# Nyrox/raymond

Hardware: AMD Instinct MI355X
Metric: Msamples/s (whole node) + achieved HBM GB/s, 1920x1080 @ 500spp 5-bounce (higher is better)
Workload: dtype f64

## Files before the change

include/raymond_hip_probe.h:

```cpp
#ifndef RAYMOND_HIP_PROBE_H
#define RAYMOND_HIP_PROBE_H

#include "raymond_hip.h"

#ifdef __cplusplus
extern "C" {
#endif

rmd_status rmd_probe_philox4x32_10(rmd_context *ctx, size_t n, const uint32_t *ctr4, const uint32_t *key2, uint32_t *out4);
rmd_status rmd_probe_block_uniforms(rmd_context *ctx, uint64_t seed, size_t n, const uint32_t *pixel, const uint32_t *sample,
                                    const uint32_t *block, double *out5);
rmd_status rmd_probe_sphere_intersect(rmd_context *ctx, size_t n, const double *sphere4, const double *ray6, int32_t *hit, double *t);
rmd_status rmd_probe_sphere_normal(rmd_context *ctx, size_t n, const double *sphere4, const double *ray6, const double *t, double *n3);
rmd_status rmd_probe_plane_intersect(rmd_context *ctx, size_t n, const double *plane6, const double *ray6, int32_t *hit, double *t);
rmd_status rmd_probe_aabb_intersect(rmd_context *ctx, size_t n, const double *aabb6, const double *ray6, int32_t *hit, double *t);
rmd_status rmd_probe_triangle_intersect(rmd_context *ctx, size_t n, const double *pos9, const double *ray6, int32_t *hit, double *t);
rmd_status rmd_probe_triangle_normal(rmd_context *ctx, size_t n, const double *pos9, const double *nrm9, const double *ray6,
                                     const double *t, double *n3);
rmd_status rmd_probe_onb(rmd_context *ctx, size_t n, const double *n3, double *t3, double *b3);
rmd_status rmd_probe_cosine_hemisphere(rmd_context *ctx, size_t n, const double *r1, const double *r2, double *dir3, double *pdf);
rmd_status rmd_probe_importance_sample_ggx(rmd_context *ctx, size_t n, const double *reflect3, const double *rough, const double *r1,
                                           const double *r2, double *dir3);
rmd_status rmd_probe_ggx_distribution(rmd_context *ctx, size_t n, const double *n3, const double *h3, const double *rough, double *out);
rmd_status rmd_probe_geometry_smith(rmd_context *ctx, size_t n, const double *n3, const double *v3, const double *l3,
                                    const double *rough, double *out);
rmd_status rmd_probe_fresnel_schlick(rmd_context *ctx, size_t n, const double *cos_theta, const double *f0_3, double *out3);
rmd_status rmd_probe_elementary(rmd_context *ctx, size_t n, const double *x, double *sqrt_out, double *sin_out, double *cos_out,
                                double *root_out, double *inv_root_out);
rmd_status rmd_probe_primary_ray(rmd_context *ctx, size_t n, const rmd_camera *cam, const uint32_t *xy2, const double *u2, double *ray6);
rmd_status rmd_probe_scene_intersect(rmd_context *ctx, const rmd_scene *scene, size_t n, const double *ray6, int32_t *obj, double *t,
                                     uint32_t *sub);
rmd_status rmd_probe_grid_intersect(rmd_context *ctx, const rmd_scene *scene, uint32_t g, size_t n, const double *ray6, int32_t *hit,
                                    double *t, uint32_t *tri);
rmd_status rmd_probe_grid_intersect_deep(rmd_context *ctx, const rmd_scene *scene, uint32_t g, size_t n, const double *ray6, uint32_t cut_lanes,
                                         uint32_t cut_round, uint32_t rays_per_wave, int32_t *hit, double *t, uint32_t *tri);
rmd_status rmd_probe_trace_samples(rmd_context *ctx, const rmd_scene *scene, const rmd_camera *cam, const rmd_settings *settings,
                                   size_t n, const uint32_t *xy2, const uint32_t *sample, double *rgb_out, int32_t *path_obj,
                                   uint32_t *path_sub);

rmd_status rmd_probe_triangle_sphere(size_t n, const double *pos9, double *out5);
rmd_status rmd_probe_primary_candidates(const rmd_camera *cam, const rmd_settings *settings, const rmd_object *objects, uint32_t n_objects, uint32_t n_grids,
                                        int64_t axis_pairs_tunable, size_t n_tiles, const uint32_t *tiles4, uint64_t *launch3, uint64_t *out2);
rmd_status rmd_probe_launch_plan(uint32_t mode, uint32_t grid, size_t n, const uint32_t *in5, uint64_t *out8);
rmd_status rmd_probe_launch_sizes(uint32_t mode, uint32_t grid, uint64_t *out8);
rmd_status rmd_probe_work_plan(const rmd_context *ctx, size_t n, const uint32_t *in4, uint32_t *out3);
rmd_status rmd_probe_work_items(uint32_t n_tiles, uint32_t n_whole, uint32_t k_tail, uint32_t sample_count, uint32_t first, size_t n, uint32_t *out5,
                                uint32_t *n_items);
rmd_status rmd_probe_scene_layout(const rmd_scene *scene, uint32_t *n_objects, uint32_t *n_grids, uint32_t *mask_words_total);
rmd_status rmd_probe_scene_plan(const rmd_scene *scene, uint64_t *out8, size_t n, uint32_t *shift_bits2);
#define RMD_PROBE_SCRATCH_FORMS 7u
#define RMD_PROBE_SCRATCH_PARTS 15u
rmd_status rmd_probe_denoise_scratch(uint32_t form, uint32_t width, uint32_t height, uint32_t n_rects, uint32_t guided, uint32_t n_cands, uint64_t n_table,
                                     uint64_t *out3, uint64_t *total);
rmd_status rmd_probe_denoise_scratch_slope(uint32_t form, uint32_t width, uint32_t height, uint32_t n_rects, uint32_t guided, uint32_t sloped, uint32_t n_cands,
                                           uint64_t n_table, uint64_t *out3, uint64_t *total);
rmd_status rmd_probe_denoise_tile(uint32_t radius, uint32_t patch_radius, uint64_t *out4);
rmd_status rmd_probe_feature_slope(rmd_context *ctx, const double *fplanes7, uint32_t width, uint32_t height, double slope, double *mplanes7);
rmd_status rmd_probe_atrous_region_slope_planes(rmd_context *ctx, uint32_t width, uint32_t height, double *mplanes7);
rmd_status rmd_probe_pretest_pairs(rmd_context *ctx, size_t n, const double *sphere5, const double *pos9, const double *ray6, int32_t *pass,
                                   int32_t *hit, double *t);

#ifdef __cplusplus
}
#endif
#endif
```

raymond_amd/csrc/api.cpp:

```cpp
#define RMD_WITH_HIP 1
#include <algorithm>
#include <cmath>
#include <limits>
#include <cstddef>
#include <cstdio>
#include <cstdlib>
#include <cstring>
#include <new>

#include "internal.hpp"
#include "launch.hpp"
#include "luma_bins.hpp"
#include "resolve_tiles_host.hpp"

using rmd::bind;

namespace {
thread_local std::string tl_last_error;

rmd_status context_create(int32_t device, hipStream_t stream, bool own_stream, rmd_context **out) {
	if (!out) return rmd::fail(nullptr, RMD_ERR_INVALID_ARGUMENT, "rmd_context_create: null out pointer");
	*out = nullptr;
	int count = 0;
	hipError_t e = hipGetDeviceCount(&count);
// ... 87 lines not shown
		RMD_HIP(ctx, hipMemcpyAsync(ctx->wave_tiles.as<rmd::WaveTile>(), wt.data(), wt.size() * sizeof(rmd::WaveTile), hipMemcpyHostToDevice, ctx->stream));
		RMD_HIP(ctx, hipStreamSynchronize(ctx->stream));
	}
	ctx->n_wave_tiles = (uint32_t)wt.size();
	ctx->cached_rects.assign(tiles, tiles + n_tiles);
	ctx->cached_W = W, ctx->cached_H = H;
	return RMD_OK;
}

rmd_status check_render_args(rmd_context *ctx, const rmd_scene *scene, const rmd_camera *cam, const rmd_settings *st) {
	if (!scene || !cam || !st) return rmd::fail(ctx, RMD_ERR_INVALID_ARGUMENT, "render: null scene/camera/settings");
	if (scene->ctx != ctx) return rmd::fail(ctx, RMD_ERR_INVALID_ARGUMENT, "render: scene belongs to another context");
	if (cam->backbuffer_width == 0 || cam->backbuffer_height == 0 || cam->backbuffer_width > 65535u || cam->backbuffer_height > 65535u)
		return rmd::fail(ctx, RMD_ERR_INVALID_ARGUMENT, "render: backbuffer size must be 1..65535 per axis");
	if (st->bounce_limit > RMD_MAX_BOUNCE_LIMIT) return rmd::fail(ctx, RMD_ERR_UNSUPPORTED, "render: bounce_limit above RMD_MAX_BOUNCE_LIMIT");
	if ((uint64_t)st->sample_begin + st->sample_count > 0xFFFFFFFFull) return rmd::fail(ctx, RMD_ERR_INVALID_ARGUMENT, "render: sample range overflows u32");
	if (st->flags & ~(RMD_RENDER_DOF | RMD_RENDER_TRACE_BLACK_PATHS | RMD_RENDER_END_BLACK_PATHS)) return rmd::fail(ctx, RMD_ERR_INVALID_ARGUMENT, "render: unknown bits in rmd_settings.flags");
	if ((st->flags & RMD_RENDER_TRACE_BLACK_PATHS) && (st->flags & RMD_RENDER_END_BLACK_PATHS))
		return rmd::fail(ctx, RMD_ERR_INVALID_ARGUMENT, "render: RMD_RENDER_TRACE_BLACK_PATHS and RMD_RENDER_END_BLACK_PATHS exclude each other");
	if (rmd::render_lds_bytes(scene->n_objects, scene->mask_words_total, 1) + (scene->n_grids == 0u ? rmd::kSortPoolBytes : 0u) > rmd::kLdsBudgetBytes)
		return rmd::fail(ctx, RMD_ERR_UNSUPPORTED, "render: object table + grid masks exceed the 160 KiB LDS of a CU");
	return RMD_OK;
}

}

namespace rmd {

rmd_status fail(rmd_context *ctx, rmd_status status, const std::string &text) {
	if (ctx) ctx->last_error = text;
	tl_last_error = text;
	return status;
}

rmd_status fail_noexcept(rmd_context *ctx, rmd_status status, const char *what, const char *text) noexcept {
	try {
		return fail(ctx, status, std::string(what) + ": " + text);
	} catch (...) {
		try {
			if (ctx) ctx->last_error.clear();
			tl_last_error.clear();
		} catch (...) {
		}
		return status;
	}
}

rmd_status bind(rmd_context *ctx) {
	if (!ctx) return fail(nullptr, RMD_ERR_INVALID_ARGUMENT, "null context");
	RMD_HIP(ctx, hipSetDevice(ctx->device));
	return RMD_OK;
}

static_assert(RMD_MAX_BOUNCE_LIMIT_DEV == RMD_MAX_BOUNCE_LIMIT, "launch.hpp mirrors include/raymond_hip.h");

rmd_status check_fault(rmd_context *ctx) {
	if (!ctx || !ctx->h_fault) return RMD_OK;
	volatile uint32_t *f = ctx->h_fault;
	const uint32_t code = f[0];
	if (code == 0u) return RMD_OK;
	const uint32_t item = f[1], reports = f[2];
	f[0] = 0u, f[1] = 0u, f[2] = 0u;
	std::string what;
	if (code & kFaultTripLoop) what += " trip loop of render_wave;";
	if (code & kFaultSortedTripLoop) what += " trip loop of render_wave_sorted;";
	if (code & kFaultWorkLoop) what += " work loop of a persistent workgroup;";
	if (code & kFaultWalkRounds) what += " round loop of a grid walk;";
	if (code & kFaultQueuedTripLoop) what += " trip loop of render_wave_queued;";
	if (code & ~(kFaultTripLoop | kFaultSortedTripLoop | kFaultWorkLoop | kFaultWalkRounds | kFaultQueuedTripLoop)) what += " unknown code;";
	char num[96];
	std::snprintf(num, sizeof(num), " %u wave(s) reported, the last one at work item %u (code 0x%x)", reports, item, code);
	return fail(ctx, RMD_ERR_DEVICE_FAULT,
	            "device fault: a loop of the render kernel ran past its bound —" + what + num +
	                "; the launch was cut short and the framebuffer it wrote to is not valid");
}

bool primary_cull_allowed(const RenderParams &P) {
	CullCamera c;
	for (int a = 0; a < 3; a++) c.pos[a] = P.cam_pos[a];
	c.width = P.width, c.height = P.height, c.aspect = P.aspect, c.tan_half_fov = P.tan_half_fov;
	return P.use_dof == 0u && cull_camera_ok(c);
}

static bool camera_on_a_plane(const rmd_scene *scene, const rmd_camera *cam) {
	for (size_t i = 0; i + 6 <= scene->planes.size(); i += 6) {
		const double *o = &scene->planes[i], *n = o + 3;
		double num = 0.0, scale = 0.0;
		for (int a = 0; a < 3; a++) num += (o[a] - cam->position[a]) * -n[a], scale += (std::fabs(o[a]) + std::fabs(cam->position[a])) * std::fabs(n[a]);
		if (!(std::fabs(num) > 1e-9 * scale)) return true;
	}
	return false;
}

RenderParams make_params(const rmd_context *ctx, const rmd_scene *scene, const rmd_camera *cam, const rmd_settings *st) {
	const double PI = 3.14159265358979323846;
	RenderParams P;
	std::memset(&P, 0, sizeof(P));
	for (int a = 0; a < 3; a++) P.cam_pos[a] = cam->position[a];
	P.width = (double)cam->backbuffer_width;
	P.height = (double)cam->backbuffer_height;
	P.inv_width = rmd::exact_reciprocal(P.width), P.inv_height = rmd::exact_reciprocal(P.height);
	P.aspect = P.width / P.height;
	P.tan_half_fov = std::tan(cam->fov_vert / 2.0 * PI / 180.0);
	P.focal_length = cam->focal_length;
	P.aperture_radius = cam->aperture_radius;
	P.W = cam->backbuffer_width, P.H = cam->backbuffer_height;
	P.bounce_limit = st->bounce_limit;
	P.sample_begin = st->sample_begin, P.sample_count = st->sample_count;
	P.n_objects = scene ? scene->n_objects : 0;
	P.n_grids = scene ? scene->n_grids : 0;
	P.mask_words_total = scene ? scene->mask_words_total : 0;
	P.key0 = (uint32_t)st->seed, P.key1 = (uint32_t)(st->seed >> 32);
	P.use_dof = ((st->flags & RMD_RENDER_DOF) && cam->aperture_radius > 0.0) ? 1u : 0u;
	const bool on_plane = scene && camera_on_a_plane(scene, cam);
	P.end_black_paths = (st->flags & RMD_RENDER_TRACE_BLACK_PATHS) ? 0u : ((st->flags & RMD_RENDER_END_BLACK_PATHS) || !scene || (scene->n_grids == 0u && scene->regular && !on_plane)) ? 1u : 0u;
	P.shade_last_depth = (scene && (!scene->regular || on_plane)) ? 1u : 0u;
	P.axis_pairs = scene ? scene->axis_pairs : 0u;
	P.visit_mask = scene ? scene->visit_mask : ~0ull, P.grid_mask = scene ? scene->grid_mask : ~0ull;
	P.primary_cull = (scene && scene->primary_cull && rmd::primary_cull_allowed(P)) ? 1u : 0u;
	P.fault = ctx ? ctx->d_fault : nullptr;
	P.walk_batch = rmd::kWalkBatchDefault;
	if (ctx && ctx->tunable[RMD_TUNE_WALK_BATCH] > 0) P.walk_batch = (uint32_t)ctx->tunable[RMD_TUNE_WALK_BATCH];
	{
		uint32_t k = rmd::kWalkCutDefault;
		if (ctx && ctx->tunable[RMD_TUNE_WALK_CUT] > 0) k = (uint32_t)std::min<int64_t>(ctx->tunable[RMD_TUNE_WALK_CUT] - 1, 31);
		P.walk_cut = (scene && scene->n_grid_objects == 1u) ? (k | (2u * k) << 8) : 0u;
		P.walk_steps_bound = scene ? scene->walk_steps_bound : 0u;
	}
#if RMD_DIAG
	if (ctx) P.debug_flags = ctx->debug_flags;
#endif
	return P;
}

}

extern "C" {

uint32_t rmd_abi_version(void) { return RMD_ABI_VERSION; }

rmd_status rmd_context_create(int32_t device_ordinal, rmd_context **out) { return context_create(device_ordinal, nullptr, true, out); }

rmd_status rmd_context_create_on_stream(int32_t device_ordinal, void *hip_stream, rmd_context **out) {
	return context_create(device_ordinal, (hipStream_t)hip_stream, false, out);
}

rmd_context::~rmd_context() {
	(void)hipSetDevice(device);
	if (stream || !owns_stream) (void)hipStreamSynchronize(stream);
	if (h_fault) (void)hipHostFree(h_fault);
	if (copy_stream) (void)hipStreamSynchronize(copy_stream);
	for (auto &sl : transfer) {
		if (sl.packed_ready) (void)hipEventDestroy(sl.packed_ready);
		if (sl.copied) (void)hipEventDestroy(sl.copied);
	}
	if (copy_stream) (void)hipStreamDestroy(copy_stream);
	if (ev_start) (void)hipEventDestroy(ev_start);
	if (ev_stop) (void)hipEventDestroy(ev_stop);
	if (owns_stream && stream) (void)hipStreamDestroy(stream);
}

void rmd_context_destroy(rmd_context *ctx) { delete ctx; }

const char *rmd_last_error(const rmd_context *ctx) { return ctx ? ctx->last_error.c_str() : tl_last_error.c_str(); }

struct GridDerived {
	std::vector<unsigned char> recs;
	std::vector<rmd::CellEntry> entries;
	std::vector<uint32_t> ids;
	std::vector<double> aux;
	std::vector<double> spheres;
	double sphere_kb = 0.0;
};
static rmd_status derive_grid_tables(rmd_context *ctx, const rmd_grid_desc &g, GridDerived &out) {
	{
		if (!g.cells || !g.mapping_table || !g.tri_pos || !g.tri_nrm || g.n_tris == 0 ||
		    g.n_cells != (uint64_t)g.resolution[0] * g.resolution[1] * g.resolution[2]) {
			return rmd::fail(ctx, RMD_ERR_INVALID_ARGUMENT, "rmd_scene_create: inconsistent grid description");
		}
		for (uint64_t c = 0; c < g.n_cells; c++) {
			uint64_t off = g.cells[c];
			if (off >= g.n_mapping || off + (uint64_t)g.mapping_table[off] >= g.n_mapping) {
				return rmd::fail(ctx, RMD_ERR_INVALID_ARGUMENT, "rmd_scene_create: cells/mapping_table run out of range");
			}
			uint32_t cnt = g.mapping_table[off];
			for (uint32_t k = 1; k <= cnt; k++)
				if (g.mapping_table[off + k] >= g.n_tris) {
					return rmd::fail(ctx, RMD_ERR_INVALID_ARGUMENT, "rmd_scene_create: triangle index out of range in mapping_table");
				}
		}
		if ((uint64_t)g.resolution[0] * ((uint64_t)g.resolution[1] + (uint64_t)g.resolution[2] * g.resolution[2]) >= (1ull << 31) ||
		    g.n_cells > (1ull << 31)) {
			return rmd::fail(ctx, RMD_ERR_UNSUPPORTED, "rmd_scene_create: grid resolution too large for 31-bit cell indices");
		}
		const uint64_t n_refs = g.n_mapping - g.n_cells;
		if (n_refs > 0xFFFFFFFFull) {
			return rmd::fail(ctx, RMD_ERR_UNSUPPORTED, "rmd_scene_create: more than 2^32-1 cell->triangle references");
		}
		std::vector<unsigned char> &recs = out.recs;
		recs.assign((size_t)g.n_tris * rmd::kTriRecStride, 0);
		for (uint64_t ti = 0; ti < g.n_tris; ti++) {
			const double *p = g.tri_pos + (size_t)ti * 9;
// ... 79 lines not shown
		if (o.material.kind != RMD_MAT_EMISSION && o.material.roughness != 0.0 && std::fabs(o.material.roughness) < rmd::kMinRoughness)
			return rmd::fail(ctx, RMD_ERR_UNSUPPORTED, "rmd_scene_create: 0 < |roughness| < 1e-12 is not supported");
		d.roughness = o.material.roughness;
		d.metalness = o.material.kind == RMD_MAT_METAL ? 1.0 : 0.0;
		{
			auto tame = [](double v) { return std::fabs(v) <= 1e150; };
			bool ok = true;
			if (o.geometry_kind != RMD_GEOM_GRID)
				for (int a = 0; a < 3; a++) ok = ok && tame(o.origin[a]);
			if (o.geometry_kind == RMD_GEOM_PLANE)
				for (int a = 0; a < 3; a++) ok = ok && tame(o.normal[a]);
			if (o.geometry_kind == RMD_GEOM_SPHERE) ok = ok && tame(o.radius) && o.radius != 0.0 && o.radius * o.radius > 0.0;
			for (int a = 0; a < 3; a++) ok = ok && tame(o.material.color[a]);
			if (o.material.kind != RMD_MAT_EMISSION) ok = ok && tame(o.material.roughness) && o.material.roughness != 0.0;
			regular = regular && ok;
		}
		if (o.material.kind == RMD_MAT_DIFFUSE && o.material.color[0] == 0.0 && o.material.color[1] == 0.0 && o.material.color[2] == 0.0) d.flags |= rmd::kObjBlackDiffuse;
	}
	for (uint32_t j = 0; j < n_objects; j++) {
		if (hobj[j].geometry_kind != RMD_GEOM_PLANE) continue;
		for (uint32_t i = 0; i < j; i++) {
			if (hobj[i].geometry_kind != RMD_GEOM_PLANE || hobj[i].pair_info != 0u) continue;
			bool opposite = true;
			for (int a = 0; a < 3; a++) opposite = opposite && hobj[j].normal[a] == -hobj[i].normal[a];
			if (!opposite) continue;
			hobj[i].pair_info = rmd::kPairTestedAtPartner | j, hobj[j].pair_info = i + 1u;
			break;
		}
	}
	uint32_t axis_pairs = 0;
	for (uint32_t j = 0; j < n_objects && j < 1023u && regular && axis_pairs_tunable != 1; j++) {
		if (hobj[j].geometry_kind != RMD_GEOM_PLANE || hobj[j].pair_info == 0u || (hobj[j].pair_info & rmd::kPairTestedAtPartner)) continue;
		const uint32_t i = hobj[j].pair_info - 1u;
		int k = -1, nonzero = 0;
		for (int a = 0; a < 3; a++)
			if (hobj[i].normal[a] != 0.0) nonzero++, k = a;
		if (nonzero != 1 || (hobj[i].normal[k] != 1.0 && hobj[i].normal[k] != -1.0) || ((axis_pairs >> (10 * k)) & 1023u) != 0u) continue;
		axis_pairs |= (j + 1u) << (10 * k);
		hobj[j].flags |= rmd::kObjAxisPair | ((uint32_t)k << rmd::kObjAxisShift) | (hobj[i].normal[k] == 1.0 ? rmd::kObjAxisEarlierIsPlus : 0u);
		hobj[i].flags |= rmd::kObjAxisPair;
		hobj[j].partner_origin_k = hobj[i].origin[k];
		hobj[j].pair_info = rmd::kPairTestedAtPartner | rmd::kPairAxis | i;
		hobj[i].pair_info |= rmd::kPairAxis;
	}
	{
		rmd::AxisWalls *walls = out.walls;
		std::memset(walls, 0, 3 * sizeof(rmd::AxisWalls));
		for (int k = 0; k < 3; k++) {
			const uint32_t f = (axis_pairs >> (10 * k)) & 1023u;
			if (f == 0u) continue;
			const uint32_t j = f - 1u, i = hobj[j].pair_info & 0x3FFFFFFFu;
			const bool e_plus = (hobj[j].flags & rmd::kObjAxisEarlierIsPlus) != 0u;
			walls[k].o_plus = e_plus ? hobj[i].origin[k] : hobj[j].origin[k], walls[k].o_minus = e_plus ? hobj[j].origin[k] : hobj[i].origin[k];
			walls[k].idx_plus = e_plus ? i : j, walls[k].idx_minus = e_plus ? j : i;
		}
	}
	out.visit_mask = 0ull, out.grid_mask = 0ull;
	for (uint32_t i = 0; i < n_objects && i < 64u; i++) {
		if (!(hobj[i].geometry_kind == RMD_GEOM_PLANE && (hobj[i].pair_info & rmd::kPairTestedAtPartner))) out.visit_mask |= 1ull << i;
		if (hobj[i].geometry_kind == RMD_GEOM_GRID) out.grid_mask |= 1ull << i;
	}
	out.regular = regular, out.axis_pairs = axis_pairs;
	return RMD_OK;
}

static rmd_status scene_create_impl(rmd_context *ctx, const rmd_object *objects, uint32_t n_objects, const rmd_grid_desc *grids, uint32_t n_grids,
                                    rmd_scene **out) {
	if (rmd_status s = bind(ctx)) return s;
	if (!out || (n_objects && !objects) || (n_grids && !grids)) return rmd::fail(ctx, RMD_ERR_INVALID_ARGUMENT, "rmd_scene_create: null argument");
	rmd::SceneObjects derived;
	if (rmd_status s = rmd::derive_scene_objects(ctx, objects, n_objects, n_grids, ctx->tunable[RMD_TUNE_AXIS_PAIRS], derived)) return s;
	std::vector<rmd::DevObject> &hobj = derived.objs;
	const bool regular = derived.regular;
	const uint32_t axis_pairs = derived.axis_pairs;
	auto sc = std::make_unique<rmd_scene>();
	sc->ctx = ctx, sc->n_objects = n_objects, sc->n_grids = n_grids, sc->regular = regular;
	sc->axis_pairs = axis_pairs;
	rmd::DevObject walls_block;
	std::memset(&walls_block, 0, sizeof(walls_block));
	std::memcpy(&walls_block, derived.walls, sizeof(derived.walls));
	sc->visit_mask = derived.visit_mask, sc->grid_mask = derived.grid_mask;
	for (uint32_t i = 0; i < n_objects; i++)
		if (objects[i].geometry_kind == RMD_GEOM_PLANE) sc->planes.insert(sc->planes.end(), objects[i].origin, objects[i].origin + 3), sc->planes.insert(sc->planes.end(), objects[i].normal, objects[i].normal + 3);
	sc->primary_cull = regular && n_grids == 0u && ctx->tunable[RMD_TUNE_AXIS_PAIRS] == 0;
	for (uint32_t i = 0; i < n_objects; i++) sc->n_grid_objects += objects[i].geometry_kind == RMD_GEOM_GRID ? 1u : 0u;
	auto upload = [&](const void *src, size_t bytes, void **dst) -> hipError_t {
		*dst = nullptr;
		rmd::DeviceBuffer b;
		hipError_t e = b.alloc(bytes ? bytes : 16);
		if (e != hipSuccess) return e;
		*dst = b.as<void>();
		sc->owned.push_back(std::move(b));
		if (bytes) e = hipMemcpy(*dst, src, bytes, hipMemcpyHostToDevice);
		return e;
	};
	std::vector<rmd::DevGrid> hgrid(n_grids);
	for (uint32_t gi = 0; gi < n_grids; gi++) {
		const rmd_grid_desc &g = grids[gi];
		rmd::DevGrid &d = hgrid[gi];
		std::memset(&d, 0, sizeof(d));
		std::shared_ptr<const GridDerived> derived;
		{
			rmd_grid_build *gb = const_cast<rmd_grid_build *>(g.built);
			const bool from_build = gb && gb->cells.data() == g.cells && gb->cells.size() == g.n_cells && gb->mapping.data() == g.mapping_table &&
			                        gb->mapping.size() == g.n_mapping && gb->pos.data() == g.tri_pos && gb->nrm.data() == g.tri_nrm && gb->pos.size() == g.n_tris * 9;
			std::unique_lock<std::mutex> lock;
			if (from_build) {
				lock = std::unique_lock<std::mutex>(gb->derived_mutex);
				derived = std::static_pointer_cast<const GridDerived>(gb->derived);
			}
			if (!derived) {
				auto fresh = std::make_shared<GridDerived>();
				if (rmd_status st = derive_grid_tables(ctx, g, *fresh)) return st;
				derived = fresh;
				if (from_build) gb->derived = fresh;
			}
		}
		const std::vector<unsigned char> &recs = derived->recs;
		const std::vector<rmd::CellEntry> &entries = derived->entries;
		const std::vector<uint32_t> &ids = derived->ids;
		const std::vector<double> &aux = derived->aux;
		for (int a = 0; a < 3; a++) {
			d.bbox_min[a] = g.bbox_min[a], d.bbox_max[a] = g.bbox_max[a], d.cell_size[a] = g.cell_size[a];
			d.inv_cell_size[a] = rmd::exact_reciprocal(g.cell_size[a]);
			d.res[a] = g.resolution[a];
			if (a == 2) sc->walk_steps_bound = std::max<uint32_t>(sc->walk_steps_bound, (uint32_t)std::min<uint64_t>((uint64_t)g.resolution[0] + g.resolution[1] + g.resolution[2] + 3u, 0xFFFFFFFFull));
		}
		d.n_cells = g.n_cells, d.n_tris = g.n_tris;
		uint64_t last_nonempty = 0;
		bool any_nonempty = false;
		for (uint64_t c = 0; c < g.n_cells; c++)
			if (entries[c * rmd::kEntrySlots].count) last_nonempty = c, any_nonempty = true;
		uint64_t covered = any_nonempty ? last_nonempty + 1 : 0;
		size_t budget_bytes = rmd::kMaskBudgetBytes;
		if (ctx->tunable[RMD_TUNE_MASK_BUDGET] > 0) budget_bytes = (size_t)ctx->tunable[RMD_TUNE_MASK_BUDGET];
		if (budget_bytes < 64) budget_bytes = 64;
		if (budget_bytes > rmd::kMaskBudgetBytes) budget_bytes = rmd::kMaskBudgetBytes;
		const size_t budget_words = budget_bytes / 4 / n_grids;
		if (budget_words < 2)
			return rmd::fail(ctx, RMD_ERR_UNSUPPORTED, "rmd_scene_create: too many grids for the LDS occupancy-mask budget");
		if ((g.n_cells + 31) / 32 + 1 <= budget_words) covered = g.n_cells;
		uint32_t shift = 0;
		while (shift < 63 && ((covered >> shift) + 31) / 32 + 1 > budget_words) shift++;
		const uint64_t bits = covered ? ((covered - 1) >> shift) + 1 : 0;
		std::vector<uint32_t> mask((size_t)((bits + 31) / 32) + 1, 0u);
		for (uint64_t c = 0; c < covered; c++)
			if (entries[c * rmd::kEntrySlots].count) mask[(c >> shift) >> 5] |= 1u << ((c >> shift) & 31u);
		d.mask_bits = (uint32_t)bits, d.mask_shift = shift, d.mask_n_words = (uint32_t)mask.size();
		d.mask_lds_word = sc->mask_words_total;
		sc->mask_words_total += (uint32_t)((mask.size() + 3) & ~(size_t)3);
		void *p = nullptr;
		RMD_HIP(ctx, upload(entries.data(), entries.size() * sizeof(rmd::CellEntry), &p));
		d.cell_entries = (const rmd::CellEntry *)p;
		RMD_HIP(ctx, upload(ids.data(), ids.size() * sizeof(uint32_t), &p));
		d.tri_ids = (const uint32_t *)p;
		RMD_HIP(ctx, upload(recs.data(), recs.size(), &p));
		d.tri_recs = p;
		RMD_HIP(ctx, upload(mask.data(), mask.size() * sizeof(uint32_t), &p));
		d.mask_words = (const uint32_t *)p;
		RMD_HIP(ctx, upload(g.tri_pos, g.n_tris * 9 * sizeof(double), &p));
		d.tri_pos = (const double *)p;
		RMD_HIP(ctx, upload(g.tri_nrm, g.n_tris * 9 * sizeof(double), &p));
		d.tri_nrm = (const double *)p;
		RMD_HIP(ctx, upload(aux.data(), aux.size() * sizeof(double), &p));
		d.tri_aux = (const double *)p;
		RMD_HIP(ctx, upload(derived->spheres.data(), derived->spheres.size() * sizeof(double), &p));
		d.tri_sph = (const double *)p, d.sph_kb = derived->sphere_kb;
// ... 53 lines not shown
}
rmd_status rmd_framebuffer_upload(rmd_context *ctx, const double *host, double *dev, size_t n) {
	if (rmd_status s = bind(ctx)) return s;
	if (!dev || !host) return rmd::fail(ctx, RMD_ERR_INVALID_ARGUMENT, "rmd_framebuffer_upload: null pointer");
	RMD_HIP(ctx, hipMemcpyAsync(dev, host, n * sizeof(double), hipMemcpyHostToDevice, ctx->stream));
	RMD_HIP(ctx, hipStreamSynchronize(ctx->stream));
	return RMD_OK;
}

static uint32_t choose_split(const rmd_context *ctx, bool has_grid, uint32_t n_wave_tiles, uint32_t sample_count, bool *buffered = nullptr) {
	uint32_t k = 1;
	bool may_buffer_unsplit = n_wave_tiles != 0 && sample_count >= (has_grid ? 1u : rmd::kSortedMinSamples);
	if (ctx->tunable[RMD_TUNE_SAMPLE_SPLIT] > 0) {
		k = (uint32_t)ctx->tunable[RMD_TUNE_SAMPLE_SPLIT];
		if (k > sample_count / 4u) k = sample_count / 4u;
		may_buffer_unsplit = false;
	} else if (n_wave_tiles != 0) {
		const uint32_t waves_per_slot = has_grid ? 256u : 24u;
		k = (waves_per_slot * ctx->wave_slots + n_wave_tiles - 1u) / n_wave_tiles;
		if (has_grid && k < 2u) k = 2u;
		uint32_t min_samples = has_grid ? (sample_count <= rmd::kChainMaxSamples && ctx->tunable[RMD_TUNE_CHAIN_ITEMS] != 1 ? 2u : rmd::kSplitMinSamplesGrid) : 64u;
		if (ctx->tunable[RMD_TUNE_SPLIT_MIN_SAMPLES] > 0) min_samples = (uint32_t)std::min<int64_t>(ctx->tunable[RMD_TUNE_SPLIT_MIN_SAMPLES], 1 << 20);
		if (k > sample_count / min_samples) k = sample_count / min_samples;
		if (has_grid && k < 2u && sample_count >= 4u && ctx->tunable[RMD_TUNE_SPLIT_MIN_SAMPLES] <= 0) k = 2u;
	}
	if (k > 64u) k = 64u;
	while (k > 1u && (uint64_t)n_wave_tiles * k > 0x7FFFFFFFull) k--;
	if (k < 2u) k = 1u;
	if (buffered) *buffered = k > 1u || may_buffer_unsplit;
	return k;
}

extern "C++" {
namespace rmd {
WorkPlan plan_work_list(uint32_t wave_slots, uint32_t n_tiles, uint32_t sample_count, uint32_t k_uniform, uint32_t min_samples, uint32_t tail_x2, uint32_t tail_parts,
                        uint32_t n_tail_forced) {
	WorkPlan w{0u, n_tiles, k_uniform < 1u ? 1u : k_uniform};
	if (tail_x2 == 0u || sample_count > kWholeMaxSamples) return w;
	const uint64_t n_tail = n_tail_forced ? (uint64_t)n_tail_forced : ((uint64_t)tail_x2 * wave_slots + 1u) / 2u;
	if ((uint64_t)n_tiles <= n_tail) return w;
	uint32_t k = tail_parts > 64u ? 64u : tail_parts;
	if (min_samples < 1u) min_samples = 1u;
	if (k > sample_count / min_samples) k = sample_count / min_samples;
	if (k < w.k_tail) k = w.k_tail;
	if ((uint64_t)(n_tiles - n_tail) + n_tail * k > 0x7FFFFFFFull) return w;
	w.n_whole = n_tiles - (uint32_t)n_tail, w.n_tail = (uint32_t)n_tail, w.k_tail = k;
	return w;
}
static WorkPlan pass_work_plan(const rmd_context *ctx, bool has_grid, bool split_launch, bool buffered, bool persistent, uint32_t n_tiles, uint32_t sample_count,
                               bool *persistent_pass) {
	WorkPlan w{0u, n_tiles, split_launch ? choose_split(ctx, has_grid, n_tiles, sample_count) : 1u};
	*persistent_pass = persistent && ((uint64_t)n_tiles * w.k_tail >= ctx->wave_slots || ctx->tunable[RMD_TUNE_LAUNCH_FORM] == 2);
	if (!buffered || has_grid || !*persistent_pass || ctx->tunable[RMD_TUNE_SAMPLE_SPLIT] > 0) return w;
	uint32_t min_samples = kTailMinSamples, forced_tail = 0u;
	if (ctx->tunable[RMD_TUNE_SPLIT_MIN_SAMPLES] > 0) min_samples = (uint32_t)std::min<int64_t>(ctx->tunable[RMD_TUNE_SPLIT_MIN_SAMPLES], 1 << 20);
#if RMD_DIAG
	if (ctx->debug_flags & 1024u) forced_tail = 4u;
#endif
	return plan_work_list(ctx->wave_slots, n_tiles, sample_count, w.k_tail, min_samples, ctx->tail_x2, ctx->tail_parts, forced_tail);
}
WorkPlan context_work_plan(const rmd_context *ctx, bool has_grid, uint32_t n_tiles, uint32_t sample_count, uint32_t pass_samples) {
	bool buffered = false, persistent_pass = false;
	const uint32_t split = choose_split(ctx, has_grid, n_tiles, sample_count, &buffered);
	return pass_work_plan(ctx, has_grid, split > 1u, buffered, ctx->tunable[RMD_TUNE_LAUNCH_FORM] != 1, n_tiles, pass_samples, &persistent_pass);
}
}
}

static rmd_status render_tiles_async_impl(rmd_context *ctx, const rmd_scene *scene, const rmd_camera *camera, const rmd_settings *settings,
                                          const rmd_tile_rect *tiles, uint32_t n_tiles, double *accum_dev, double *accum_sq_dev) {
	if (rmd_status s = bind(ctx)) return s;
	if (rmd_status s = check_render_args(ctx, scene, camera, settings)) return s;
	if (!accum_dev || (n_tiles && !tiles)) return rmd::fail(ctx, RMD_ERR_INVALID_ARGUMENT, "rmd_render_tiles: null tiles/accum pointer");
	if (rmd_status s = prepare_wave_tiles(ctx, camera, tiles, n_tiles)) return s;
	if (settings->bounce_limit == 0u) {
		RMD_HIP(ctx, hipEventRecord(ctx->ev_start, ctx->stream));
		RMD_HIP(ctx, hipEventRecord(ctx->ev_stop, ctx->stream));
		ctx->timed = true;
		return RMD_OK;
	}
	rmd::RenderParams P = rmd::make_params(ctx, scene, camera, settings);
	P.n_work = ctx->n_wave_tiles;
	if (P.debug_flags & 24u) {
		RMD_HIP(ctx, ctx->debug_counters.grow(48 * sizeof(unsigned long long)));
		RMD_HIP(ctx, hipMemsetAsync(ctx->debug_counters.as<void>(), 0, 48 * sizeof(unsigned long long), ctx->stream));
		P.debug_counters = ctx->debug_counters.as<unsigned long long>();
	}
	bool buffered = false;
	uint32_t split = choose_split(ctx, scene->n_grids != 0, P.n_work, P.sample_count, &buffered);
	const bool persistent = ctx->tunable[RMD_TUNE_LAUNCH_FORM] != 1;
	if (persistent) RMD_HIP(ctx, ctx->work_counter.grow(256));
	uint32_t per_pass = P.sample_count;
	if (buffered) {
		const size_t bytes_per_sample = (size_t)P.n_work * 64u * rmd::kSampleStride * sizeof(double);
		size_t cap;
		if (ctx->tunable[RMD_TUNE_SCRATCH_CAP_MB] > 0) cap = (size_t)ctx->tunable[RMD_TUNE_SCRATCH_CAP_MB] << 20;
		else {
			size_t free_b = 0, total_b = 0;
			RMD_HIP(ctx, hipMemGetInfo(&free_b, &total_b));
			cap = (free_b + ctx->sample_buf.bytes()) / 8;
		}
		if (bytes_per_sample * per_pass > cap) per_pass = (uint32_t)(cap / bytes_per_sample);
		const uint64_t sectors_per_sample = (uint64_t)P.n_work * 64u;
		if (sectors_per_sample * per_pass > 0xFFFFFFFFull) per_pass = (uint32_t)(0xFFFFFFFFull / sectors_per_sample);
		if (per_pass < 8u) per_pass = 8u;
		if (per_pass > P.sample_count) per_pass = P.sample_count;
		if (sectors_per_sample * per_pass > 0xFFFFFFFFull) split = 1u, buffered = false, per_pass = P.sample_count;
		while (buffered && bytes_per_sample * per_pass > ctx->sample_buf.bytes()) {
			rmd::DeviceBuffer fresh;
			const hipError_t e = fresh.alloc(bytes_per_sample * per_pass);
			if (e == hipSuccess) {
				ctx->sample_buf = std::move(fresh);
				break;
			}
			(void)hipGetLastError();
			if (e != hipErrorOutOfMemory) return rmd::fail(ctx, RMD_ERR_HIP, std::string("hipMalloc(sample scratch): ") + hipGetErrorString(e));
			if (per_pass <= 8u) {
				split = 1u, buffered = false, per_pass = P.sample_count;
				break;
			}
			per_pass = per_pass / 2u < 8u ? 8u : per_pass / 2u;
		}
	}
	ctx->last_launch = rmd_launch_info{};
	ctx->last_launch.end_black_paths = P.end_black_paths, ctx->last_launch.has_grid = scene->n_grids != 0u;
	RMD_HIP(ctx, hipEventRecord(ctx->ev_start, ctx->stream));
	for (uint64_t done = 0; done < settings->sample_count || done == 0; done += per_pass) {
		rmd::RenderParams Q = P;
		Q.sample_begin = settings->sample_begin + (uint32_t)done;
		Q.sample_count = settings->sample_count - done < per_pass ? (uint32_t)(settings->sample_count - done) : per_pass;
		bool persistent_pass = false;
		const rmd::WorkPlan list = rmd::pass_work_plan(ctx, scene->n_grids != 0, split > 1u, buffered, persistent, P.n_work, Q.sample_count, &persistent_pass);
		Q.split_k = list.k_tail, Q.n_whole = list.n_whole;
		Q.sample_magic = Q.sample_count > 1u ? ~0ull / Q.sample_count + 1ull : 0ull;
		Q.buffered = buffered ? 1u : 0u;
		{
			const int64_t force = ctx->tunable[RMD_TUNE_CHAIN_ITEMS];
			Q.chain_items = (buffered && scene->n_grids != 0u && (force == 2 || (force == 0 && Q.sample_count <= rmd::kChainMaxSamples))) ? 1u : 0u;
		}
		Q.sample_buf = ctx->sample_buf.as<double>();
		if (persistent_pass) {
			RMD_HIP(ctx, hipMemsetAsync(ctx->work_counter.as<void>(), 0, sizeof(uint32_t), ctx->stream));
			Q.work_counter = ctx->work_counter.as<uint32_t>();
		}
		if (persistent_pass && buffered && scene->n_grids != 0u && ctx->tunable[RMD_TUNE_PATH_QUEUES] != 1) {
			const size_t wave_bytes = rmd::path_queue_bytes_host(rmd::kQueuePaths), need = wave_bytes * ctx->wave_slots;
			if (ctx->queue_buf.bytes() < need) {
				const hipError_t qe = (ctx->debug_flags & 256u) ? hipErrorOutOfMemory : ctx->queue_buf.grow(need);
				if (qe == hipSuccess) {
					RMD_HIP(ctx, hipMemsetAsync(ctx->queue_buf.as<void>(), 0, need, ctx->stream));
				} else {
					(void)hipGetLastError();
					if (qe != hipErrorOutOfMemory) return rmd::fail(ctx, RMD_ERR_HIP, std::string("hipMalloc(path queues): ") + hipGetErrorString(qe));
				}
			}
			if (ctx->queue_buf.bytes()) Q.queue_buf = ctx->queue_buf.as<unsigned char>(), Q.queue_wave_bytes = (uint32_t)wave_bytes, Q.queue_paths = rmd::kQueuePaths;
		}
		if (buffered && scene->n_grids == 0) {
			RMD_HIP(ctx, ctx->tile_done.grow((size_t)P.n_work * sizeof(uint32_t)));
			RMD_HIP(ctx, hipMemsetAsync(ctx->tile_done.as<void>(), 0, (size_t)P.n_work * sizeof(uint32_t), ctx->stream));
			Q.tile_done = ctx->tile_done.as<uint32_t>();
		}
		rmd::LaunchShape shape;
		RMD_HIP(ctx, rmd::launch_render_tiles(ctx->stream, Q, scene->d_objects, scene->d_grids, ctx->wave_tiles.as<rmd::WaveTile>(), accum_dev, persistent_pass ? ctx->n_cus : 0u, &shape,
		                                      accum_sq_dev));
		ctx->last_launch.passes++, ctx->last_launch.split_k = Q.split_k, ctx->last_launch.buffered = Q.buffered;
		ctx->last_launch.persistent = shape.persistent, ctx->last_launch.waves_per_workgroup = shape.waves_per_wg;
		ctx->last_launch.queued = shape.queued;
		ctx->last_launch.chained = shape.chained;
		if (settings->sample_count == 0) break;
	}
	RMD_HIP(ctx, hipEventRecord(ctx->ev_stop, ctx->stream));
	ctx->timed = true;
	if (P.debug_flags & 24u) {
		unsigned long long h[48];
		RMD_HIP(ctx, hipMemcpyAsync(h, ctx->debug_counters.as<void>(), sizeof(h), hipMemcpyDeviceToHost, ctx->stream));
		RMD_HIP(ctx, hipStreamSynchronize(ctx->stream));
		if ((P.debug_flags & 16u) && ctx->last_launch.queued) {
			static const char *kinds[3] = {"GEN  ", "SHADE", "WALK "};
			for (int k = 0; k < 3; k++)
				std::fprintf(stderr, "[rmd queued stamps, cycles] %s trips=%llu fetch=%llu make_ray=%llu simple=%llu walk=%llu ray_push=%llu classify=%llu stores=%llu\n", kinds[k], h[k * 8 + 7],
				             h[k * 8 + 0], h[k * 8 + 1], h[k * 8 + 2], h[k * 8 + 3], h[k * 8 + 4], h[k * 8 + 5], h[k * 8 + 6]);
			std::fprintf(stderr, "[rmd queued stamps, cycles] inside the walks: init=%llu stepping=%llu entry_wait=%llu scan=%llu (chunk search+load+test)=%llu hits=%llu tail=%llu\n",
			             h[24], h[25], h[26], h[27], h[29], h[30], h[31]);
		} else if (P.debug_flags & 16u)
			std::fprintf(stderr, "[rmd stamps, cycles] wave_total=%llu next_ray=%llu simple=%llu walk=%llu classify=%llu | walk: init=%llu stepping=%llu entry_wait=%llu scan=%llu (chunk search+load+test)=%llu hits=%llu tail=%llu\n",
			             h[0], h[1], h[2], h[3], h[4], h[8], h[9], h[10], h[11], h[13], h[14], h[15]);
		else
			std::fprintf(stderr, "[rmd debug] walk_calls=%llu walkers=%llu calls_with_walkers=%llu rounds=%llu wave_steps=%llu lane_steps=%llu test_rounds=%llu tests=%llu chunks=%llu | main_iterations=%llu live_lanes=%llu lanes_with_ray=%llu | stepping iterations with <= 4 / 8 / 16 lanes: %llu / %llu / %llu, with <= 8 lanes while tests wait: %llu\n",
			             h[0], h[1], h[2], h[3], h[4], h[5], h[6], h[8], h[9], h[10], h[11], h[12], h[7], h[13], h[14], h[15]);
		if ((P.debug_flags & 16u) == 0u)
			std::fprintf(stderr, "[rmd debug] sphere pre-test: pairs passed=%llu full chunks=%llu | pairs dropped that pass the reference's test (flag 64; must be 0)=%llu\n", h[17], h[18], h[16]);
		if ((P.debug_flags & 16u) == 0u && (P.debug_flags & 512u))
			std::fprintf(stderr, "[rmd debug] primary candidates: lanes checked=%llu sphere turns left out=%llu trips with two axis pairs left out=%llu | cleared spheres that register a hit (must be 0)=%llu closest hits that differ from the full visit's (must be 0)=%llu\n",
			             h[32], h[35], h[36], h[33], h[34]);
		if ((P.debug_flags & 16u) == 0u && ctx->last_launch.buffered && scene->n_grids == 0u)
			std::fprintf(stderr, "[rmd debug] lobe trips: diffuse trips=%llu diffuse hits shaded=%llu ggx trips=%llu ggx hits shaded=%llu | hits parked: diffuse=%llu ggx=%llu\n", h[37], h[38], h[39],
			             h[40], h[41], h[42]);
		if ((P.debug_flags & 16u) == 0u && ctx->last_launch.queued)
			std::fprintf(stderr, "[rmd debug] path queues: rays pushed=%llu (of them walks put aside=%llu) rays held in their lanes=%llu hits pushed=%llu hits held in their lanes=%llu\n", h[19], h[22], h[23], h[20], h[21]);
	}
	return RMD_OK;
}

rmd_status rmd_render_tiles_async(rmd_context *ctx, const rmd_scene *scene, const rmd_camera *camera, const rmd_settings *settings,
                                  const rmd_tile_rect *tiles, uint32_t n_tiles, double *accum_dev) {
	return rmd::guarded(ctx, "rmd_render_tiles", [&] { return render_tiles_async_impl(ctx, scene, camera, settings, tiles, n_tiles, accum_dev, nullptr); });
}

rmd_status rmd_render_tiles_moments_async(rmd_context *ctx, const rmd_scene *scene, const rmd_camera *camera, const rmd_settings *settings,
                                          const rmd_tile_rect *tiles, uint32_t n_tiles, double *accum_dev, double *accum_sq_dev) {
	if (accum_sq_dev != nullptr && accum_sq_dev == accum_dev)
		return rmd::fail(ctx, RMD_ERR_INVALID_ARGUMENT, "rmd_render_tiles_moments: accum_sq_dev must not alias accum_dev");
	return rmd::guarded(ctx, "rmd_render_tiles_moments",
	                    [&] { return render_tiles_async_impl(ctx, scene, camera, settings, tiles, n_tiles, accum_dev, accum_sq_dev); });
}

rmd_status rmd_context_set_tunable(rmd_context *ctx, uint32_t key, int64_t value) {
	if (!ctx) return rmd::fail(nullptr, RMD_ERR_INVALID_ARGUMENT, "rmd_context_set_tunable: null context");
	if (key >= RMD_TUNE_COUNT || value < 0) return rmd::fail(ctx, RMD_ERR_INVALID_ARGUMENT, "rmd_context_set_tunable: unknown key or negative value");
	if (key == RMD_TUNE_LAUNCH_FORM && value > 2) return rmd::fail(ctx, RMD_ERR_INVALID_ARGUMENT, "rmd_context_set_tunable: launch form is 0 .. 2");
	ctx->tunable[key] = value;
	return RMD_OK;
}
rmd_status rmd_context_get_tunable(const rmd_context *ctx, uint32_t key, int64_t *out_value) {
	if (!ctx || !out_value || key >= RMD_TUNE_COUNT) return rmd::fail(nullptr, RMD_ERR_INVALID_ARGUMENT, "rmd_context_get_tunable: bad argument");
	*out_value = ctx->tunable[key];
	return RMD_OK;
}

rmd_status rmd_context_memory_info(rmd_context *ctx, uint64_t *out_free_bytes, uint64_t *out_total_bytes) {
	if (rmd_status s = bind(ctx)) return s;
	if (!out_free_bytes || !out_total_bytes) return rmd::fail(ctx, RMD_ERR_INVALID_ARGUMENT, "rmd_context_memory_info: null pointer");
	size_t free_b = 0, total_b = 0;
	RMD_HIP(ctx, hipMemGetInfo(&free_b, &total_b));
	*out_free_bytes = free_b, *out_total_bytes = total_b;
	return RMD_OK;
}

rmd_status rmd_context_synchronize(rmd_context *ctx) {
	if (rmd_status s = bind(ctx)) return s;
	RMD_HIP(ctx, hipStreamSynchronize(ctx->stream));
	return rmd::check_fault(ctx);
}

rmd_status rmd_render_tiles(rmd_context *ctx, const rmd_scene *scene, const rmd_camera *camera, const rmd_settings *settings,
                            const rmd_tile_rect *tiles, uint32_t n_tiles, double *accum_dev) {
	if (rmd_status s = rmd_render_tiles_async(ctx, scene, camera, settings, tiles, n_tiles, accum_dev)) return s;
	return rmd_context_synchronize(ctx);
}

rmd_status rmd_render_tiles_moments(rmd_context *ctx, const rmd_scene *scene, const rmd_camera *camera, const rmd_settings *settings,
                                    const rmd_tile_rect *tiles, uint32_t n_tiles, double *accum_dev, double *accum_sq_dev) {
	if (rmd_status s = rmd_render_tiles_moments_async(ctx, scene, camera, settings, tiles, n_tiles, accum_dev, accum_sq_dev)) return s;
	return rmd_context_synchronize(ctx);
}

static rmd_status tile_error_impl(rmd_context *ctx, const double *accum_dev, const double *accum_sq_dev, uint32_t width, uint32_t height,
                                  uint32_t sample_count, double floor, const rmd_tile_rect *rects, uint32_t n_rects, double *out_err_host) {
	if (rmd_status s = bind(ctx)) return s;
	for (uint32_t i = 0; i < n_rects; i++)
		if ((uint64_t)rects[i].left + rects[i].width > width || (uint64_t)rects[i].top + rects[i].height > height)
			return rmd::fail(ctx, RMD_ERR_INVALID_ARGUMENT, "rmd_tile_error: tile rectangle outside the framebuffer");
	rmd::DeviceBuffer d;
	if (n_rects != 0) {
		const size_t rect_bytes = (size_t)n_rects * sizeof(rmd_tile_rect);
		RMD_HIP(ctx, d.alloc(rect_bytes + (size_t)n_rects * sizeof(double)));
		rmd_tile_rect *d_rects = d.as<rmd_tile_rect>();
		double *d_err = reinterpret_cast<double *>(d.as<unsigned char>() + rect_bytes);
		RMD_HIP(ctx, hipMemcpyAsync(d_rects, rects, rect_bytes, hipMemcpyHostToDevice, ctx->stream));
		RMD_HIP(ctx, rmd::launch_tile_error(ctx->stream, accum_dev, accum_sq_dev, d_rects, n_rects, width, sample_count, floor, d_err));
		RMD_HIP(ctx, hipMemcpyAsync(out_err_host, d_err, (size_t)n_rects * sizeof(double), hipMemcpyDeviceToHost, ctx->stream));
	}
	RMD_HIP(ctx, hipStreamSynchronize(ctx->stream));
	return rmd::check_fault(ctx);
}

rmd_status rmd_tile_error(rmd_context *ctx, const double *accum_dev, const double *accum_sq_dev, uint32_t width, uint32_t height, uint32_t sample_count,
                          double floor, const rmd_tile_rect *rects, uint32_t n_rects, double *out_err_host) {
	if (!accum_dev || !accum_sq_dev || width == 0 || height == 0 || (n_rects && (!rects || !out_err_host)))
		return rmd::fail(ctx, RMD_ERR_INVALID_ARGUMENT, "rmd_tile_error: bad argument");
// ... 417 lines not shown
```

raymond_amd/csrc/internal.hpp:

```cpp
#pragma once
#include <stdint.h>

#include <cmath>
#include <limits>
#include <algorithm>
#include <cstring>

#include <memory>
#include <mutex>
#include <string>
#include <vector>

#include "../../include/raymond_hip.h"

#ifdef RMD_WITH_HIP
#include <hip/hip_runtime_api.h>

#include "device_types.hpp"
#include "primary_candidates.hpp"
#include "work_list.hpp"

#define RMD_HIP(ctx, call)                                                                                      \
	do {                                                                                                        \
		hipError_t e_ = (call);                                                                                 \
// ... 4 lines not shown
namespace rmd {
class DeviceBuffer {
public:
	DeviceBuffer() = default;
	DeviceBuffer(DeviceBuffer &&o) noexcept : p_(o.p_), bytes_(o.bytes_) { o.p_ = nullptr, o.bytes_ = 0; }
	DeviceBuffer &operator=(DeviceBuffer &&o) noexcept {
		if (this != &o) (void)release(), p_ = o.p_, bytes_ = o.bytes_, o.p_ = nullptr, o.bytes_ = 0;
		return *this;
	}
	~DeviceBuffer() { (void)release(); }
	hipError_t release() {
		const hipError_t e = p_ ? hipFree(p_) : hipSuccess;
		p_ = nullptr, bytes_ = 0;
		return e;
	}
	hipError_t alloc(size_t bytes) {
		hipError_t e = release();
		if (e == hipSuccess) e = hipMalloc(&p_, bytes);
		if (e == hipSuccess) bytes_ = bytes;
		else p_ = nullptr;
		return e;
	}
	hipError_t grow(size_t bytes) { return bytes <= bytes_ ? hipSuccess : alloc(bytes); }
	size_t bytes() const { return bytes_; }
	template <class T>
	T *as() const { return static_cast<T *>(p_); }

private:
	void *p_ = nullptr;
	size_t bytes_ = 0;
};
}

struct rmd_context {
	int device = 0;
	hipStream_t stream = nullptr;
	bool owns_stream = false;
	hipEvent_t ev_start = nullptr, ev_stop = nullptr;
	bool timed = false;
	std::string last_error;
	std::vector<rmd_tile_rect> cached_rects;
	uint32_t cached_W = 0, cached_H = 0;
	rmd::DeviceBuffer wave_tiles;
	uint32_t n_wave_tiles = 0;
	rmd::DeviceBuffer sample_buf;
	uint32_t wave_slots = 0;
	uint32_t n_cus = 0;
	rmd::DeviceBuffer work_counter;
	rmd::DeviceBuffer queue_buf;
	rmd::DeviceBuffer tile_done;
	rmd::DeviceBuffer debug_counters;
	rmd::DeviceBuffer atrous_region_scratch;
	size_t atrous_region_slope_offset = 0, atrous_region_slope_pixels = 0;
	rmd::DeviceBuffer resolve_tiles_scratch;
	std::vector<unsigned char> resolve_tiles_table;
	rmd::DeviceBuffer luma_scratch;
	std::vector<unsigned char> luma_table;
	rmd::DeviceBuffer despike_scratch;
	uint32_t *h_fault = nullptr, *d_fault = nullptr;
	struct TransferSlot {
		rmd::DeviceBuffer packed;
		rmd::DeviceBuffer table;
		hipEvent_t packed_ready = nullptr, copied = nullptr;
		bool in_flight = false;
		std::vector<unsigned char> h_table;
	} transfer[2];
	uint32_t next_transfer = 0;
	hipStream_t copy_stream = nullptr;
	int64_t tunable[RMD_TUNE_COUNT] = {};
	uint32_t debug_flags = 0;
	uint32_t tail_x2 = rmd::kTailTilesPerSlotX2, tail_parts = rmd::kTailParts;
	rmd_launch_info last_launch = {};
	~rmd_context();
};

struct rmd_scene {
	rmd_context *ctx = nullptr;
	uint32_t n_objects = 0, n_grids = 0;
	uint32_t n_grid_objects = 0;
	uint32_t mask_words_total = 0;
	uint32_t axis_pairs = 0;
	unsigned long long visit_mask = ~0ull, grid_mask = ~0ull;
	uint32_t walk_steps_bound = 0;
	bool primary_cull = false;
	bool regular = true;
	std::vector<double> planes;
	rmd::DevObject *d_objects = nullptr;
	rmd::DevGrid *d_grids = nullptr;
	std::vector<rmd::DeviceBuffer> owned;
	~rmd_scene();
};
#endif

struct rmd_grid_build {
	double bbox_min[3], bbox_max[3], cell_size[3];
	uint32_t res[3];
	std::vector<uint32_t> cells, mapping;
	std::vector<double> pos, nrm;
	std::shared_ptr<void> derived;
	std::mutex derived_mutex;
};

namespace rmd {
inline void mesh_bounds(const double *tri_pos, uint64_t n_tris, double bbox_min[3], double bbox_max[3]) {
	static const double seed_min[3] = {125125.0, 1251251.0, 12512512.0}, seed_max[3] = {-123125.0, -125123.0, -512123.0};
	for (int a = 0; a < 3; a++) bbox_min[a] = seed_min[a], bbox_max[a] = seed_max[a];
	for (uint64_t i = 0; i < n_tris * 3; i++)
		for (int a = 0; a < 3; a++) {
			const double v = tri_pos[i * 3 + a];
			if (v <= bbox_min[a]) bbox_min[a] = v;
			if (v >= bbox_max[a]) bbox_max[a] = v;
		}
}
inline double exact_reciprocal(double b) {
	uint64_t bits;
	std::memcpy(&bits, &b, 8);
	const double m = std::fabs(b);
	if (!(m >= 0x1p-500 && m <= 0x1p500) || (bits & 0xFFFFFFFFFFFFFull) == 0xFFFFFFFFFFFFFull) return std::nan("");
	return 1.0 / b;
}
inline void triangle_sphere(const double *p9, double out[4], double &kb) {
	const double *P[3] = {p9, p9 + 3, p9 + 6};
	auto sub = [](const double *a, const double *b, double *o) { for (int i = 0; i < 3; i++) o[i] = a[i] - b[i]; };
	auto dot = [](const double *a, const double *b) { return a[0] * b[0] + a[1] * b[1] + a[2] * b[2]; };
	auto cross = [](const double *a, const double *b, double *o) { o[0] = a[1] * b[2] - a[2] * b[1], o[1] = a[2] * b[0] - a[0] * b[2], o[2] = a[0] * b[1] - a[1] * b[0]; };
	double e[3][3], l2[3];
	sub(P[2], P[1], e[0]), sub(P[0], P[2], e[1]), sub(P[1], P[0], e[2]);
	for (int i = 0; i < 3; i++) l2[i] = dot(e[i], e[i]);
	const int longest = l2[0] >= l2[1] && l2[0] >= l2[2] ? 0 : (l2[1] >= l2[2] ? 1 : 2);
	const double L = std::sqrt(l2[longest]);
	double c[3];
	for (int i = 0; i < 3; i++) c[i] = 0.5 * (P[(longest + 1) % 3][i] + P[(longest + 2) % 3][i]);
	double dv[3];
	sub(P[longest], c, dv);
	if (dot(dv, dv) > 0.25 * l2[longest]) {
		double a[3], b[3], n[3], t1[3], t2[3];
		sub(P[1], P[0], a), sub(P[2], P[0], b), cross(a, b, n);
		const double n2 = dot(n, n);
		cross(n, a, t1), cross(b, n, t2);
		if (n2 > 0.0 && std::isfinite(n2))
			for (int i = 0; i < 3; i++) c[i] = P[0][i] + (dot(b, b) * t1[i] + dot(a, a) * t2[i]) / (2.0 * n2);
	}
	double r2 = 0.0;
	for (int v = 0; v < 3; v++) {
		sub(P[v], c, dv);
		r2 = std::max(r2, dot(dv, dv));
	}
	const double cmax = std::max(std::fabs(c[0]), std::max(std::fabs(c[1]), std::fabs(c[2])));
	const double r = std::sqrt(r2) * 1.001 + 4.4e-6 * L * L * L + 1e-12 * (1.0 + cmax);
	out[0] = c[0], out[1] = c[1], out[2] = c[2], out[3] = 1.01 * r * r;
	const double k = 4.4e-6 * L * L;
	kb = 101.0 * k * k + 32.0 * 2.220446049250313e-16;
	if (!(std::isfinite(out[0]) && std::isfinite(out[1]) && std::isfinite(out[2]) && std::isfinite(out[3]) && std::isfinite(kb)))
		out[0] = out[1] = out[2] = 0.0, out[3] = std::numeric_limits<double>::infinity(), kb = 0.0;
}
inline void triangle_aux(const double *p9, double out[4]) {
	auto dist = [](const double *a, const double *b) {
		const double dx = b[0] - a[0], dy = b[1] - a[1], dz = b[2] - a[2];
		return std::sqrt((dx * dx + dy * dy) + dz * dz);
	};
	const double ab = dist(p9, p9 + 3), ac = dist(p9, p9 + 6), bc = dist(p9 + 3, p9 + 6);
	const double s = (ab + ac + bc) / 2.0;
	out[0] = ab, out[1] = ac, out[2] = std::sqrt(s * (s - ab) * (s - ac) * (s - bc)), out[3] = exact_reciprocal(out[2]);
}
rmd_status fail(rmd_context *ctx, rmd_status status, const std::string &text);
rmd_status fail_noexcept(rmd_context *ctx, rmd_status status, const char *what, const char *text) noexcept;
template <class F>
rmd_status guarded(rmd_context *ctx, const char *what, F &&body) noexcept {
	try {
		return body();
	} catch (const std::bad_alloc &) {
		return fail_noexcept(ctx, RMD_ERR_OUT_OF_MEMORY, what, "the host ran out of memory");
	} catch (const std::exception &e) {
		return fail_noexcept(ctx, RMD_ERR_HIP, what, e.what());
	} catch (...) {
		return fail_noexcept(ctx, RMD_ERR_HIP, what, "unknown exception");
	}
}
#ifdef RMD_WITH_HIP
rmd_status bind(rmd_context *ctx);
bool denoise_rects_ok(const rmd_tile_rect *rects, uint32_t n_rects, uint32_t width, uint32_t height, const char **why);
rmd_status check_fault(rmd_context *ctx);
RenderParams make_params(const rmd_context *ctx, const rmd_scene *scene, const rmd_camera *cam, const rmd_settings *st);
bool primary_cull_allowed(const RenderParams &P);
WorkPlan plan_work_list(uint32_t wave_slots, uint32_t n_tiles, uint32_t sample_count, uint32_t k_uniform, uint32_t min_samples = kTailMinSamples,
                        uint32_t tail_x2 = kTailTilesPerSlotX2, uint32_t tail_parts = kTailParts, uint32_t n_tail_forced = 0u);
WorkPlan context_work_plan(const rmd_context *ctx, bool has_grid, uint32_t n_tiles, uint32_t sample_count, uint32_t pass_samples);
struct SceneObjects {
	std::vector<DevObject> objs;
	bool regular = true;
	uint32_t axis_pairs = 0;
	AxisWalls walls[3] = {};
	unsigned long long visit_mask = 0ull, grid_mask = 0ull;
};
rmd_status derive_scene_objects(rmd_context *ctx, const rmd_object *objects, uint32_t n_objects, uint32_t n_grids, int64_t axis_pairs_tunable, SceneObjects &out);
#endif
}
```

raymond_amd/csrc/primary_candidates.hpp:

```cpp
#pragma once
#include <stdint.h>

#include "device_types.hpp"

#if defined(__HIP__)
#define RMD_HD __host__ __device__ inline
#else
#define RMD_HD inline
#endif

namespace rmd {

constexpr double kCullWiden = 1e-9;
constexpr double kCullSphereMargin = 3200.0 * 2.220446049250313e-16;
constexpr double kCullFacing = 2e-6;
constexpr double kCullPairMargin = 1e-9;

struct CullCamera {
	double pos[3];
	double width, height, aspect, tan_half_fov;
};
struct TileCone {
	double lo[2], hi[2];
	double a[3];
	double cos_t, sin_t;
	double u_max;
	bool ok;
};
RMD_HD double cull_abs(double v) { return v < 0.0 ? -v : v; }
RMD_HD double cull_min(double a, double b) { return a < b ? a : b; }
RMD_HD double cull_max(double a, double b) { return a > b ? a : b; }

RMD_HD bool cull_camera_ok(const CullCamera &c) {
	const double big = 1e150;
	bool ok = cull_abs(c.pos[0]) <= big && cull_abs(c.pos[1]) <= big && cull_abs(c.pos[2]) <= big;
	ok = ok && c.tan_half_fov > 0.0 && c.tan_half_fov <= big && c.aspect > 0.0 && c.aspect <= big;
	return ok && c.width > 0.0 && c.width <= big && c.height > 0.0 && c.height <= big;
}

RMD_HD TileCone primary_tile_cone(const CullCamera &c, uint32_t x0, uint32_t y0, uint32_t w, uint32_t h) {
	TileCone T;
	const double ex = c.tan_half_fov * c.aspect, ey = c.tan_half_fov;
	const double pxa = (2.0 * ((double)x0 / c.width) - 1.0) * ex, pxb = (2.0 * ((double)(x0 + w) / c.width) - 1.0) * ex;
	const double pya = (1.0 - 2.0 * ((double)y0 / c.height)) * ey, pyb = (1.0 - 2.0 * ((double)(y0 + h) / c.height)) * ey;
	T.lo[0] = cull_min(pxa, pxb) - kCullWiden * ex, T.hi[0] = cull_max(pxa, pxb) + kCullWiden * ex;
	T.lo[1] = cull_min(pya, pyb) - kCullWiden * ey, T.hi[1] = cull_max(pya, pyb) + kCullWiden * ey;
	const double cx = 0.5 * (T.lo[0] + T.hi[0]), cy = 0.5 * (T.lo[1] + T.hi[1]);
	const double cl = __builtin_sqrt((cx * cx + cy * cy) + 1.0);
	T.a[0] = cx / cl, T.a[1] = cy / cl, T.a[2] = 1.0 / cl;
	double cos_t = 1.0, sin_t = 0.0, u_max = 1.0;
	for (int k = 0; k < 4; k++) {
		const double qx = (k & 1) ? T.hi[0] : T.lo[0], qy = (k & 2) ? T.hi[1] : T.lo[1];
		const double ql = __builtin_sqrt((qx * qx + qy * qy) + 1.0);
		const double dx = qx / ql, dy = qy / ql, dz = 1.0 / ql;
		const double cs = (T.a[0] * dx + T.a[1] * dy) + T.a[2] * dz;
		const double kx = T.a[1] * dz - T.a[2] * dy, ky = T.a[2] * dx - T.a[0] * dz, kz = T.a[0] * dy - T.a[1] * dx;
		const double sn = __builtin_sqrt((kx * kx + ky * ky) + kz * kz);
		cos_t = cull_min(cos_t, cs), sin_t = cull_max(sin_t, sn), u_max = cull_max(u_max, ql);
	}
	T.cos_t = cos_t, T.sin_t = sin_t, T.u_max = u_max;
	T.ok = cos_t > 0.7072 && sin_t < 0.7072 && u_max < 1e150 && T.lo[0] > -1e150 && T.hi[0] < 1e150 && T.lo[1] > -1e150 && T.hi[1] < 1e150;
	return T;
}

RMD_HD bool primary_sphere_cleared(const TileCone &T, const CullCamera &c, const double centre[3], double radius) {
	if (!T.ok) return false;
	const double vx = centre[0] - c.pos[0], vy = centre[1] - c.pos[1], vz = centre[2] - c.pos[2];
	const double va = (vx * T.a[0] + vy * T.a[1]) + vz * T.a[2];
	const double kx = vy * T.a[2] - vz * T.a[1], ky = vz * T.a[0] - vx * T.a[2], kz = vx * T.a[1] - vy * T.a[0];
	const double vxa = __builtin_sqrt((kx * kx + ky * ky) + kz * kz);
	const double r = cull_abs(radius);
	const double K = ((cull_abs(vx) + cull_abs(vy)) + cull_abs(vz)) + ((cull_abs(centre[0]) + cull_abs(centre[1])) + cull_abs(centre[2])) +
	                 ((cull_abs(c.pos[0]) + cull_abs(c.pos[1])) + cull_abs(c.pos[2])) + r;
	const double margin = kCullSphereMargin * K;
	const bool in_front = va * T.cos_t - vxa * T.sin_t > margin;
	const double D = vxa * T.cos_t - va * T.sin_t;
	return in_front && D > r + margin && K <= 1e150;
}

RMD_HD uint32_t primary_pairs_kept(const TileCone &T, const CullCamera &c, const AxisWalls walls[3], uint32_t axis_pairs) {
	if (!T.ok) return axis_pairs;
	double s_lo[3], s_hi[3];
	bool paired[3];
	for (int k = 0; k < 3; k++) {
		paired[k] = ((axis_pairs >> (10 * k)) & 1023u) != 0u;
		s_lo[k] = 0.0, s_hi[k] = -1.0;
		if (!paired[k]) continue;
		const double num_plus = c.pos[k] - walls[k].o_plus, num_minus = walls[k].o_minus - c.pos[k];
		if (!(num_plus > 0.0 && num_minus > 0.0)) return axis_pairs;
		const double lo = k < 2 ? T.lo[k] : 1.0, hi = k < 2 ? T.hi[k] : 1.0;
		double nearest = 1e300;
		if (hi > 0.0) nearest = cull_min(nearest, num_minus / hi);
		if (lo < 0.0) nearest = cull_min(nearest, num_plus / -lo);
		s_lo[k] = nearest;
		if (!(s_lo[k] > 0.0)) return axis_pairs;
		const bool pos = lo > 0.0, neg = hi < 0.0;
		if (pos || neg) {
			const double u_lo = pos ? lo : -hi;
			if (u_lo > kCullFacing * T.u_max) s_hi[k] = (pos ? num_minus : num_plus) / u_lo;
		}
	}
	for (int k = 0; k < 3; k++) {
		if (!paired[k] || !(s_hi[k] > 0.0)) continue;
		bool alone = true;
		for (int j = 0; j < 3; j++)
			if (j != k && paired[j]) alone = alone && s_hi[k] * (1.0 + kCullPairMargin) < s_lo[j];
		if (alone) return axis_pairs & (1023u << (10 * k));
	}
	return axis_pairs;
}

}
```

raymond_amd/csrc/probe.cpp:

```cpp
#define RMD_WITH_HIP 1
#include <cstring>
#include <vector>

#include "../../include/raymond_hip_probe.h"
#include "internal.hpp"
#include "launch.hpp"

namespace {

struct Column {
	const double *src;
	int width;
};

rmd_status run_probe(rmd_context *ctx, int op, size_t n, const std::vector<Column> &cols, int out_stride, std::vector<double> &out,
                     const rmd::RenderParams *params = nullptr) {
	if (!ctx) return rmd::fail(nullptr, RMD_ERR_INVALID_ARGUMENT, "probe: null context");
	RMD_HIP(ctx, hipSetDevice(ctx->device));
	int in_stride = 0;
	for (const Column &c : cols) {
		if (!c.src && n) return rmd::fail(ctx, RMD_ERR_INVALID_ARGUMENT, "probe: null input array");
		in_stride += c.width;
	}
	std::vector<double> in(n * in_stride);
// ... 141 lines not shown
rmd_status rmd_probe_primary_ray(rmd_context *ctx, size_t n, const rmd_camera *cam, const uint32_t *xy2, const double *u2, double *ray6) {
	if (!cam || !xy2) return rmd::fail(ctx, RMD_ERR_INVALID_ARGUMENT, "probe: null argument");
	rmd_settings st;
	std::memset(&st, 0, sizeof(st));
	rmd::RenderParams P = rmd::make_params(ctx, nullptr, cam, &st);
	std::vector<double> xy = widen(xy2, n * 2), out;
	if (rmd_status s = run_probe(ctx, rmd::PROBE_PRIMARY_RAY, n, {{xy.data(), 2}, {u2, 2}}, 6, out, &P)) return s;
	unpack(out, 6, 0, 6, ray6, n);
	return RMD_OK;
}

static rmd_status scene_probe(rmd_context *ctx, const rmd_scene *scene, int mode, uint32_t g, size_t n, const double *ray6, int32_t *a,
                              double *t, uint32_t *b) {
	if (!ctx || !scene || scene->ctx != ctx || !ray6 || !a || !t || !b) return rmd::fail(ctx, RMD_ERR_INVALID_ARGUMENT, "probe: bad argument");
	if (mode == 1 && g >= scene->n_grids) return rmd::fail(ctx, RMD_ERR_INVALID_ARGUMENT, "probe: grid index out of range");
	RMD_HIP(ctx, hipSetDevice(ctx->device));
	if (n == 0) return RMD_OK;
	rmd::DeviceBuffer din, dout;
	RMD_HIP(ctx, din.alloc(n * 6 * sizeof(double)));
	RMD_HIP(ctx, dout.alloc(n * 3 * sizeof(double)));
	RMD_HIP(ctx, hipMemcpyAsync(din.as<void>(), ray6, n * 6 * sizeof(double), hipMemcpyHostToDevice, ctx->stream));
	RMD_HIP(ctx, rmd::launch_probe_scene(ctx->stream, mode, g, (uint32_t)n, scene->d_objects, scene->n_objects, scene->d_grids,
	                                     scene->n_grids, scene->mask_words_total, scene->axis_pairs, din.as<const double>(), dout.as<double>()));
	std::vector<double> out(n * 3);
	RMD_HIP(ctx, hipMemcpyAsync(out.data(), dout.as<void>(), out.size() * sizeof(double), hipMemcpyDeviceToHost, ctx->stream));
	RMD_HIP(ctx, hipStreamSynchronize(ctx->stream));
	for (size_t i = 0; i < n; i++) a[i] = (int32_t)out[3 * i], t[i] = out[3 * i + 1], b[i] = (uint32_t)out[3 * i + 2];
	return RMD_OK;
}

rmd_status rmd_probe_scene_intersect(rmd_context *ctx, const rmd_scene *scene, size_t n, const double *ray6, int32_t *obj, double *t,
                                     uint32_t *sub) {
	return scene_probe(ctx, scene, 0, 0, n, ray6, obj, t, sub);
}
rmd_status rmd_probe_grid_intersect(rmd_context *ctx, const rmd_scene *scene, uint32_t g, size_t n, const double *ray6, int32_t *hit,
                                    double *t, uint32_t *tri) {
	return scene_probe(ctx, scene, 1, g, n, ray6, hit, t, tri);
}

rmd_status rmd_probe_grid_intersect_deep(rmd_context *ctx, const rmd_scene *scene, uint32_t g, size_t n, const double *ray6, uint32_t cut_lanes,
                                         uint32_t cut_round, uint32_t rays_per_wave, int32_t *hit, double *t, uint32_t *tri) {
	if (!ctx || !scene || scene->ctx != ctx || !ray6 || !hit || !t || !tri) return rmd::fail(ctx, RMD_ERR_INVALID_ARGUMENT, "probe: bad argument");
	if (g >= scene->n_grids) return rmd::fail(ctx, RMD_ERR_INVALID_ARGUMENT, "probe: grid index out of range");
	if (rays_per_wave == 0u || rays_per_wave % 64u != 0u || rays_per_wave > (1u << 20) || cut_lanes > 255u || cut_round > 255u || n > 0x7FFFFFFFull)
		return rmd::fail(ctx, RMD_ERR_INVALID_ARGUMENT, "probe: rays_per_wave must be a multiple of 64 up to 2^20, the cuts at most 255, n below 2^31");
	RMD_HIP(ctx, hipSetDevice(ctx->device));
	if (n == 0) return RMD_OK;
	rmd::DeviceBuffer din, dout, dstuck;
	RMD_HIP(ctx, din.alloc(n * 6 * sizeof(double)));
	RMD_HIP(ctx, dout.alloc(n * 3 * sizeof(double)));
	RMD_HIP(ctx, dstuck.alloc(sizeof(uint32_t)));
	RMD_HIP(ctx, hipMemcpyAsync(din.as<void>(), ray6, n * 6 * sizeof(double), hipMemcpyHostToDevice, ctx->stream));
	RMD_HIP(ctx, hipMemsetAsync(dout.as<void>(), 0, n * 3 * sizeof(double), ctx->stream));
	RMD_HIP(ctx, hipMemsetAsync(dstuck.as<void>(), 0, sizeof(uint32_t), ctx->stream));
	RMD_HIP(ctx, rmd::launch_probe_grid_deep(ctx->stream, g, (uint32_t)n, scene->d_grids, scene->n_grids, scene->mask_words_total, din.as<const double>(), cut_lanes,
	                                         cut_round, rays_per_wave, scene->walk_steps_bound, dout.as<double>(), dstuck.as<uint32_t>()));
	std::vector<double> out(n * 3);
	uint32_t stuck = 0;
	RMD_HIP(ctx, hipMemcpyAsync(out.data(), dout.as<void>(), out.size() * sizeof(double), hipMemcpyDeviceToHost, ctx->stream));
	RMD_HIP(ctx, hipMemcpyAsync(&stuck, dstuck.as<void>(), sizeof(uint32_t), hipMemcpyDeviceToHost, ctx->stream));
	RMD_HIP(ctx, hipStreamSynchronize(ctx->stream));
	if (stuck) return rmd::fail(ctx, RMD_ERR_DEVICE_FAULT, "probe: a wave of the DEEP walk reached its bound of walk calls with rays unfinished (it cannot: an internal fault)");
	for (size_t i = 0; i < n; i++) hit[i] = (int32_t)out[3 * i], t[i] = out[3 * i + 1], tri[i] = (uint32_t)out[3 * i + 2];
	return RMD_OK;
}

rmd_status rmd_probe_triangle_sphere(size_t n, const double *pos9, double *out5) {
	if (n != 0 && (!pos9 || !out5)) return rmd::fail(nullptr, RMD_ERR_INVALID_ARGUMENT, "probe: bad argument");
	for (size_t i = 0; i < n; i++) {
		double kb = 0.0;
		rmd::triangle_sphere(pos9 + i * 9, out5 + i * 5, kb);
		out5[i * 5 + 4] = kb;
	}
	return RMD_OK;
}

rmd_status rmd_probe_primary_candidates(const rmd_camera *cam, const rmd_settings *settings, const rmd_object *objects, uint32_t n_objects, uint32_t n_grids,
                                        int64_t axis_pairs_tunable, size_t n_tiles, const uint32_t *tiles4, uint64_t *launch3, uint64_t *out2) {
	if (!cam || !settings || (n_objects && !objects) || !launch3 || (n_tiles != 0 && (!tiles4 || !out2))) return rmd::fail(nullptr, RMD_ERR_INVALID_ARGUMENT, "probe: bad argument");
	return rmd::guarded(nullptr, "rmd_probe_primary_candidates", [&]() -> rmd_status {
		rmd::SceneObjects sc;
		if (rmd_status s = rmd::derive_scene_objects(nullptr, objects, n_objects, n_grids, axis_pairs_tunable, sc)) return s;
		const rmd::RenderParams P = rmd::make_params(nullptr, nullptr, cam, settings);
		const bool on = sc.regular && n_grids == 0u && axis_pairs_tunable == 0 && rmd::primary_cull_allowed(P);
		launch3[0] = sc.visit_mask, launch3[1] = sc.axis_pairs, launch3[2] = on ? 1u : 0u;
		rmd::CullCamera cc;
		for (int a = 0; a < 3; a++) cc.pos[a] = P.cam_pos[a];
		cc.width = P.width, cc.height = P.height, cc.aspect = P.aspect, cc.tan_half_fov = P.tan_half_fov;
		for (size_t i = 0; i < n_tiles; i++) {
			const uint32_t *t = tiles4 + i * 4;
			uint64_t visit = sc.visit_mask;
			uint32_t pairs = sc.axis_pairs;
			if (on) {
				if (t[2] == 0u || t[2] > 8u || t[3] == 0u || t[3] > 8u || t[0] > 65535u || t[1] > 65535u) return rmd::fail(nullptr, RMD_ERR_INVALID_ARGUMENT, "probe: a wave tile is 1..8 pixels a side");
				const rmd::TileCone cone = rmd::primary_tile_cone(cc, t[0], t[1], t[2], t[3]);
				for (uint32_t j = 0; j < n_objects && j < 64u; j++)
					if (sc.objs[j].geometry_kind == 1u && rmd::primary_sphere_cleared(cone, cc, sc.objs[j].origin, sc.objs[j].radius)) visit &= ~(1ull << j);
				pairs = rmd::primary_pairs_kept(cone, cc, sc.walls, sc.axis_pairs);
			}
			out2[i * 2] = visit, out2[i * 2 + 1] = pairs;
		}
		return RMD_OK;
	});
}

rmd_status rmd_probe_launch_plan(uint32_t mode, uint32_t grid, size_t n, const uint32_t *in5, uint64_t *out8) {
	if (mode > 2u || grid > 1u || (n != 0 && (!in5 || !out8))) return rmd::fail(nullptr, RMD_ERR_INVALID_ARGUMENT, "probe: bad argument");
	for (size_t i = 0; i < n; i++) {
		const uint32_t *a = in5 + i * 5;
		const rmd::LaunchPlan L = rmd::plan_render_launch((int)mode, grid != 0u, a[0], a[1], (a[2] & 1u) != 0u, (a[2] & 2u) != 0u, (a[2] & 4u) != 0u,
		                                                  (a[2] & 8u) != 0u, a[3], a[4]);
		uint64_t *o = out8 + i * 8;
		o[0] = L.persistent, o[1] = L.queued, o[2] = L.chained, o[3] = L.moments, o[4] = L.waves_per_wg, o[5] = L.workgroups, o[6] = L.wave_lds, o[7] = L.lds;
	}
	return RMD_OK;
}

rmd_status rmd_probe_work_plan(const rmd_context *ctx, size_t n, const uint32_t *in4, uint32_t *out3) {
	if (n != 0 && (!in4 || !out3)) return rmd::fail(nullptr, RMD_ERR_INVALID_ARGUMENT, "probe: bad argument");
	for (size_t i = 0; i < n; i++) {
		const uint32_t *a = in4 + i * 4;
		const rmd::WorkPlan w = ctx ? rmd::context_work_plan(ctx, false, a[1], a[2], a[0] ? a[0] : a[2]) : rmd::plan_work_list(a[0], a[1], a[2], a[3]);
		out3[i * 3] = w.n_whole, out3[i * 3 + 1] = w.n_tail, out3[i * 3 + 2] = w.k_tail;
	}
	return RMD_OK;
}

rmd_status rmd_probe_work_items(uint32_t n_tiles, uint32_t n_whole, uint32_t k_tail, uint32_t sample_count, uint32_t first, size_t n, uint32_t *out5,
                                uint32_t *n_items) {
	if (n_whole > n_tiles || k_tail == 0u || !n_items || (n != 0 && !out5)) return rmd::fail(nullptr, RMD_ERR_INVALID_ARGUMENT, "probe: bad argument");
	*n_items = rmd::work_list_items(n_tiles, n_whole, k_tail);
	for (size_t i = 0; i < n; i++) {
		const rmd::WorkItem w = rmd::work_list_item(first + (uint32_t)i, n_tiles, n_whole, k_tail, sample_count);
		uint32_t *o = out5 + i * 5;
		o[0] = w.tile, o[1] = w.first, o[2] = w.count, o[3] = w.parts, o[4] = w.whole;
	}
	return RMD_OK;
}

rmd_status rmd_probe_launch_sizes(uint32_t mode, uint32_t grid, uint64_t *out8) {
	if (mode > 2u || grid > 1u || !out8) return rmd::fail(nullptr, RMD_ERR_INVALID_ARGUMENT, "probe: bad argument");
	rmd::render_lds_sizes((int)mode, grid != 0u, out8);
	return RMD_OK;
}

static_assert(RMD_PROBE_SCRATCH_FORMS == rmd::kScratchForms && RMD_PROBE_SCRATCH_PARTS == rmd::kScratchParts, "include/raymond_hip_probe.h mirrors denoise_host.hpp");
rmd_status rmd_probe_denoise_scratch(uint32_t form, uint32_t width, uint32_t height, uint32_t n_rects, uint32_t guided, uint32_t n_cands, uint64_t n_table,
                                     uint64_t *out3, uint64_t *total) {
	if (form >= rmd::kScratchForms || guided > 1u || !out3 || !total) return rmd::fail(nullptr, RMD_ERR_INVALID_ARGUMENT, "probe: bad argument");
	const rmd::ScratchLayout L = rmd::denoise_scratch_layout((rmd::ScratchForm)form, width, height, n_rects, guided != 0u, n_cands, (size_t)n_table);
	for (uint32_t p = 0; p < rmd::kScratchParts; p++) out3[3 * p] = L.used[p], out3[3 * p + 1] = L.offset[p], out3[3 * p + 2] = L.bytes[p];
	*total = L.total;
	return RMD_OK;
}
rmd_status rmd_probe_denoise_scratch_slope(uint32_t form, uint32_t width, uint32_t height, uint32_t n_rects, uint32_t guided, uint32_t sloped, uint32_t n_cands,
                                           uint64_t n_table, uint64_t *out3, uint64_t *total) {
	if (form >= rmd::kScratchForms || guided > 1u || sloped > 2u || !out3 || !total) return rmd::fail(nullptr, RMD_ERR_INVALID_ARGUMENT, "probe: bad argument");
	const rmd::ScratchLayout L = rmd::denoise_scratch_layout((rmd::ScratchForm)form, width, height, n_rects, guided != 0u, n_cands, (size_t)n_table, sloped == 1u, sloped == 2u);
	for (uint32_t p = 0; p < rmd::kScratchParts; p++) out3[3 * p] = L.used[p], out3[3 * p + 1] = L.offset[p], out3[3 * p + 2] = L.bytes[p];
	*total = L.total;
	return RMD_OK;
}

rmd_status rmd_probe_denoise_tile(uint32_t radius, uint32_t patch_radius, uint64_t *out4) {
	if (radius > rmd::kDenoiseMaxRadius || patch_radius > rmd::kDenoiseMaxPatch || !out4) return rmd::fail(nullptr, RMD_ERR_INVALID_ARGUMENT, "probe: bad argument");
	const uint32_t tw = rmd::denoise_tile_width(radius, patch_radius);
	out4[0] = tw, out4[1] = rmd::denoise_lds_bytes(tw, radius, patch_radius), out4[2] = rmd::denoise_lds_bytes(32u, radius, patch_radius), out4[3] = rmd::kLdsBudgetBytes;
	return RMD_OK;
}

rmd_status rmd_probe_feature_slope(rmd_context *ctx, const double *fplanes7, uint32_t width, uint32_t height, double slope, double *mplanes7) {
	if (!ctx || !fplanes7 || !mplanes7 || width == 0 || height == 0) return rmd::fail(ctx, RMD_ERR_INVALID_ARGUMENT, "probe: bad argument");
	RMD_HIP(ctx, hipSetDevice(ctx->device));
	const size_t bytes = (size_t)width * height * RMD_FEATURE_CHANNELS * sizeof(double);
	rmd::DeviceBuffer df, dm;
	RMD_HIP(ctx, df.alloc(bytes));
	RMD_HIP(ctx, dm.alloc(bytes));
	RMD_HIP(ctx, hipMemcpyAsync(df.as<void>(), fplanes7, bytes, hipMemcpyHostToDevice, ctx->stream));
	RMD_HIP(ctx, rmd::launch_feature_slope(ctx->stream, df.as<double>(), width, height, slope, dm.as<double>()));
	RMD_HIP(ctx, hipMemcpyAsync(mplanes7, dm.as<void>(), bytes, hipMemcpyDeviceToHost, ctx->stream));
	RMD_HIP(ctx, hipStreamSynchronize(ctx->stream));
	return RMD_OK;
}

rmd_status rmd_probe_atrous_region_slope_planes(rmd_context *ctx, uint32_t width, uint32_t height, double *mplanes7) {
	if (!ctx || !mplanes7 || ctx->atrous_region_slope_pixels == 0u || (size_t)width * height != ctx->atrous_region_slope_pixels)
		return rmd::fail(ctx, RMD_ERR_INVALID_ARGUMENT, "probe: bad argument");
	RMD_HIP(ctx, hipSetDevice(ctx->device));
// ... 73 lines not shown
```

raymond_amd/csrc/render_kernel.hpp:

```cpp
#pragma once
#include <hip/hip_runtime.h>

#include "device_core.hpp"
#include "grid_walk.hpp"
#include "launch.hpp"
#include "lobe_trips.hpp"
#include "primary_candidates.hpp"
#include "scene_split.hpp"
#include "work_list.hpp"

namespace rmd {

struct alignas(16) PathId {
	uint32_t px[64];
	uint32_t smp[64];
	uint32_t sector[64];
};
__host__ __device__ inline size_t wave_lds_bytes(uint32_t n_grids) { return kWaveHeadBytes + (n_grids ? sizeof(WalkScratch) + 64u * 3u * sizeof(double) + sizeof(WalkCarry) + sizeof(PathId) : 0); }

RMD_DEV uint32_t work_item_of_block(uint32_t b, uint32_t nb) {
	(void)nb;
	return b;
}

RMD_DEV void report_fault(const RenderParams &P, uint32_t code, uint32_t detail) {
	if ((threadIdx.x & 63u) == 0u) {
		if (P.fault != nullptr) {
			__hip_atomic_fetch_or(P.fault, code, __ATOMIC_RELAXED, __HIP_MEMORY_SCOPE_SYSTEM);
			__hip_atomic_store(P.fault + 1, detail, __ATOMIC_RELAXED, __HIP_MEMORY_SCOPE_SYSTEM);
			__hip_atomic_fetch_add(P.fault + 2, 1u, __ATOMIC_RELAXED, __HIP_MEMORY_SCOPE_SYSTEM);
		}
		if (P.work_counter != nullptr) __hip_atomic_fetch_or(P.work_counter, kWorkCounterPoison, __ATOMIC_RELAXED, __HIP_MEMORY_SCOPE_AGENT);
	}
}
constexpr uint32_t kTripBoundPerPair = RMD_MAX_BOUNCE_LIMIT_DEV + 4u;
constexpr uint32_t kStallBound = 1u << 18;

template <bool GRID>
RMD_DEV int scene_intersect_wave(const DevObject *__restrict__ objs, uint32_t n_objects, const DevGrid *__restrict__ grids,
                                 const uint32_t *lds_masks, WalkScratch &scr, bool want, V3 ro, V3 rd, double &t_best, uint32_t &sub_best,
                                 uint32_t axis_pairs, uint32_t debug_flags = 0, unsigned long long *dbg = nullptr, bool arbitrary_rays = false,
                                 unsigned long long turns = ~0ull) {
	double closest = kFMax;
	int best = -1;
	uint32_t sub = 0;
	axis_pairs_visit(objs, n_objects, axis_pairs, want, ro, rd, closest, best, arbitrary_rays);
	if constexpr (!GRID) {
		for (uint32_t i = next_turn(~0u, turns); i < n_objects; i = next_turn(i, turns)) {
			const DevObject &o = objs[i];
			double t;
			bool ok;
			int idx = (int)i;
			if (o.geometry_kind == 0u) {
				if (o.pair_info != 0u) {
					if (o.pair_info & kPairTestedAtPartner) continue;
					const uint32_t e = o.pair_info - 1u;
					bool first;
					ok = plane_pair_test_flat(ld3(objs[e].origin), ld3(objs[e].normal), ld3(o.origin), ld3(o.normal), ro, rd, t, first);
					idx = first ? (int)e : (int)i;
					ok = ok && want && lex_less(t, idx, closest, best);
				} else {
					ok = plane_test_flat(ld3(o.origin), ld3(o.normal), ro, rd, t) && want && lex_less(t, idx, closest, best);
				}
			} else {
				ok = sphere_test_flat(ld3(o.origin), o.radius, ro, rd, t) && want && lex_less(t, idx, closest, best);
			}
			closest = ok ? t : closest, best = ok ? idx : best;
		}
		t_best = closest, sub_best = 0u;
		return best;
	}
	for (uint32_t i = next_turn(~0u, turns); i < n_objects; i = next_turn(i, turns)) {
		const DevObject &o = objs[i];
		if (o.geometry_kind == 0u) {
			if (o.pair_info != 0u) {
				const uint32_t e = o.pair_info - 1u;
				if (want && (o.pair_info & kPairTestedAtPartner) == 0u)
					plane_pair_visit(ld3(objs[e].origin), ld3(objs[e].normal), ld3(o.origin), ld3(o.normal), ro, rd, [&](double t, bool first) {
						const int idx = first ? (int)e : (int)i;
						if (lex_less(t, idx, closest, best)) closest = t, best = idx, sub = 0u;
					});
			} else if (want)
				plane_visit(ld3(o.origin), ld3(o.normal), ro, rd, [&](double t) {
					if (lex_less(t, (int)i, closest, best)) closest = t, best = (int)i, sub = 0u;
				});
		} else if (o.geometry_kind == 1u) {
			if (want)
				sphere_visit(ld3(o.origin), o.radius, ro, rd, [&](double t) {
					if (lex_less(t, (int)i, closest, best)) closest = t, best = (int)i, sub = 0u;
				});
		} else if constexpr (GRID) {
			const DevGrid &g = grids[o.grid_index];
			const uint32_t *mask = (lds_masks && g.mask_lds_word != 0xFFFFFFFFu) ? lds_masks + g.mask_lds_word : nullptr;
			double t;
			uint32_t tri = 0;
			bool hit = false;
			grid_intersect_wave(g, mask, scr, want, ro, rd, hit, t, tri, debug_flags, dbg);
			if (want && hit && lex_less(t, (int)i, closest, best)) closest = t, best = (int)i, sub = tri;
		}
	}
	t_best = closest;
	sub_best = sub;
	return best;
}

constexpr uint32_t kWalkMinRunnable = 24;
constexpr uint32_t kWalkMaxWait = 6;
constexpr uint32_t kWalkCutMinWalkers = 16;
constexpr uint32_t kWalkCutMinRunnable = 0;

constexpr uint32_t kGridMinWaves = 4, kNoGridMinWaves = 3;
enum { kModeTiles = 0, kModeTilesBuffered = 1, kModeList = 2 };
RMD_DEV void store_sample(RMD_GLOBAL double *dst, V3 L) { dst[0] = L.x, dst[1] = L.y, dst[2] = L.z; }
template <bool MOM = false>
RMD_DEV void finish_sample_range(const RenderParams &P, const WaveTile &tile, uint32_t wt, uint32_t parts, bool whole, uint32_t lane, double *__restrict__ out,
                                 double *__restrict__ out_sq = nullptr) {
	if (P.tile_done == nullptr || wt >= P.n_work) return;
	if (whole) {
		__builtin_amdgcn_fence(__ATOMIC_RELEASE, "wavefront");
		__builtin_amdgcn_s_waitcnt(0);
		__builtin_amdgcn_wave_barrier();
		__builtin_amdgcn_fence(__ATOMIC_ACQUIRE, "wavefront");
	} else {
		__builtin_amdgcn_fence(__ATOMIC_RELEASE, "agent");
		uint32_t before = 0;
		if (lane == 0u) before = __hip_atomic_fetch_add(P.tile_done + wt, 1u, __ATOMIC_RELAXED, __HIP_MEMORY_SCOPE_AGENT);
		before = (uint32_t)__builtin_amdgcn_readfirstlane((int)before);
		if (before + 1u != parts) return;
		__builtin_amdgcn_fence(__ATOMIC_ACQUIRE, "agent");
	}
	const uint32_t lx = lane & 7u, ly = lane >> 3;
	if (lx < tile.w && ly < tile.h) {
		const size_t pix = ((size_t)(tile.x0 + lx) + (size_t)(tile.y0 + ly) * P.W) * 3;
		V3 sum = ld3(out + pix);
		[[maybe_unused]] V3 sq = mk(0.0, 0.0, 0.0);
		if constexpr (MOM) sq = ld3(out_sq + pix);
		const RMD_GLOBAL double *src = (const RMD_GLOBAL double *)P.sample_buf + ((size_t)wt * P.sample_count * 64u + lane) * kSampleStride;
		constexpr uint32_t kInFlight = MOM ? 8u : 16u;
		uint32_t k = 0;
		for (; k + kInFlight <= P.sample_count; k += kInFlight) {
			V3 v[kInFlight];
#pragma unroll
			for (uint32_t j = 0; j < kInFlight; j++) v[j] = ld3(src + (size_t)j * 64u * kSampleStride);
#pragma unroll
			for (uint32_t j = 0; j < kInFlight; j++) {
				sum = sum + v[j];
				if constexpr (MOM) sq = sq + hadamard(v[j], v[j]);
			}
			src += kInFlight * 64u * kSampleStride;
		}
		for (; k < P.sample_count; k++) {
			const V3 v = ld3(src);
			sum = sum + v;
			if constexpr (MOM) sq = sq + hadamard(v, v);
			src += 64u * kSampleStride;
		}
		out[pix + 0] = sum.x, out[pix + 1] = sum.y, out[pix + 2] = sum.z;
		if constexpr (MOM) out_sq[pix + 0] = sq.x, out_sq[pix + 1] = sq.y, out_sq[pix + 2] = sq.z;
	}
}

typedef const __attribute__((address_space(4))) unsigned long long *KernargWords;
template <int MODE, bool GRID, bool CHAIN = false, bool MOM = false>
RMD_DEV void render_wave(const RenderParams &P, KernargWords kernarg_params, const DevObject *__restrict__ objs, const DevGrid *__restrict__ grids,
                         const void *__restrict__ work, double *__restrict__ out, int32_t *__restrict__ path_obj, uint32_t *__restrict__ path_sub,
                         const DevObject *lobjs, const uint32_t *lds_masks, unsigned char *wave_lds, uint32_t first, double *__restrict__ out_sq = nullptr) {
	static_assert(!CHAIN || (MODE == kModeTilesBuffered && GRID), "items are chained in split launches of scenes with grids");
	static_assert(!MOM || MODE == kModeTiles, "split launches add the squares where they add the samples (finish_sample_range, sum_moments_kernel)");
	constexpr bool LIST = MODE == kModeList;
	const uint32_t lane = threadIdx.x & 63u;
	WalkScratch &scr = *reinterpret_cast<WalkScratch *>(wave_lds);

	constexpr bool to_buffer = MODE == kModeTilesBuffered;
	uint32_t x = 0, y = 0, s = 0, s_end = 0;
	bool alive = false;
	size_t out_index = 0;
	uint32_t list_idx = 0;
	WaveTile tile = {};
	uint32_t wt = 0, pool_first = 0, pool_items = 0, next_item = 0;
	uint32_t item = 0;
	constexpr bool id_in_lds = to_buffer && GRID;
	[[maybe_unused]] PathId *pid = GRID ? reinterpret_cast<PathId *>(wave_lds + sizeof(WalkScratch) + 64u * 3u * sizeof(double) + sizeof(WalkCarry)) : nullptr;
	if (LIST) {
		list_idx = first + lane;
		alive = list_idx < P.n_work;
		ListWork w = reinterpret_cast<const ListWork *>(work)[alive ? list_idx : 0];
		x = w.x, y = w.y, s = w.sample, s_end = w.sample + 1u;
		out_index = (size_t)list_idx * 3;
	} else {
		const uint32_t work_item = first;
		const uint32_t split = to_buffer ? P.split_k : 1u;
		wt = work_item / split;
		const uint32_t part = work_item % split;
		const bool have = wt < P.n_work;
		tile = reinterpret_cast<const WaveTile *>(work)[have ? wt : 0];
		const uint32_t per_part = (P.sample_count + split - 1u) / split;
		const uint32_t s_lo = part * per_part < P.sample_count ? part * per_part : P.sample_count;
		const uint32_t s_hi = s_lo + per_part < P.sample_count ? s_lo + per_part : P.sample_count;
		if constexpr (to_buffer) {
			pool_first = s_lo;
			pool_items = have ? (s_hi - s_lo) * 64u : 0u;
		} else {
			const uint32_t lx = lane & 7u, ly = lane >> 3;
			alive = have && lx < tile.w && ly < tile.h && s_hi > s_lo;
			x = tile.x0 + lx, y = tile.y0 + ly;
			s = P.sample_begin + s_lo, s_end = P.sample_begin + s_hi;
			out_index = ((size_t)x + (size_t)y * P.W) * 3;
		}
	}
	const bool writes = alive;

	constexpr bool acc_in_memory = GRID && MODE == kModeTiles;
	V3 acc = mk(0.0, 0.0, 0.0);
	if (!LIST && alive && !to_buffer && !acc_in_memory) acc = ld3(out + out_index);
	[[maybe_unused]] V3 acc_sq = mk(0.0, 0.0, 0.0);
	if constexpr (MOM && !acc_in_memory)
		if (alive) acc_sq = ld3(out_sq + out_index);
	if (P.bounce_limit == 0u) {
		if (LIST && writes) out[out_index + 0] = 0.0, out[out_index + 1] = 0.0, out[out_index + 2] = 0.0;
		return;
// ... 229 lines not shown
			hit.normal = hit_normal;
			hit.frag = ro + rd * hit_t;
			hit.color = ld3(o.color), hit.roughness = o.roughness, hit.metal = o.metalness;
		}
		[[maybe_unused]] bool black = false;
		if constexpr (GRID) {
			V3 T = mk(1.0, 1.0, 1.0);
			if (to_shade) T = load_T();
			next_ray(Pt, to_shade, prim, hit, cam_pos, x, y, rng, ro, rd, T);
			if (to_shade || prim) store_T(T);
			black = Pt.end_black_paths != 0u && T.x == 0.0 && T.y == 0.0 && T.z == 0.0;
		} else {
			next_ray(Pt, to_shade, prim, hit, cam_pos, x, y, rng, ro, rd, T_reg);
			black = Pt.end_black_paths != 0u && T_reg.x == 0.0 && T_reg.y == 0.0 && T_reg.z == 0.0;
		}
		if (Pt.use_dof) {
			if (prim) lens_failed = !thin_lens_from_pinhole(Pt, ro, rd, rng, ro, rd);
		}
		rng_block = rng.block, lobe_bits = rng.lobe_bits;
		cut = false;
		if (to_shade) {
			depth++;
			to_shade = false;
			if (depth > Pt.bounce_limit || (!LIST && black)) cut = true, has_ray = false;
			else has_ray = true, new_ray = true;
		}
#if RMD_DIAG
		if ((Pt.debug_flags & 8u) && Pt.debug_counters) {
			const unsigned long long am = __ballot(alive), wm = __ballot(has_ray && !lens_failed);
			if (lane == 0) atomicAdd(&Pt.debug_counters[10], 1ull), atomicAdd(&Pt.debug_counters[11], (unsigned long long)__popcll(am)), atomicAdd(&Pt.debug_counters[12], (unsigned long long)__popcll(wm));
		}
#endif
		RMD_TSTAMP(tt_b)
		const bool want = has_ray && !lens_failed;
		if constexpr (GRID) {
			if (want && new_ray) {
				waiting = intersect_simple(objs, Pt.n_objects, grids, true, ro, rd, part_t, part_obj, Pt.axis_pairs, Pt.visit_mask);
				part_sub = 0u, new_ray = false;
			}
			RMD_TSTAMP(tt_simple)
			const unsigned long long wm = __ballot(want && waiting), rm = __ballot(alive && !(want && waiting));
			if ((trips_since_walk & 0xFFu) != 0xFFu) trips_since_walk++;
			if (wm != 0ull && ((uint32_t)__popcll(wm) >= Pt.walk_batch || (uint32_t)__popcll(rm) < kWalkMinRunnable || (trips_since_walk & 0xFFu) >= kWalkMaxWait)) {
				trips_since_walk &= ~0xFFu;
				if constexpr (MODE != kModeTiles) {
					const uint32_t n_walkers = (uint32_t)__popcll(wm);
					const bool cut = n_walkers >= kWalkCutMinWalkers && (uint32_t)__popcll(rm) >= kWalkCutMinRunnable;
					const uint32_t cut_lanes = cut ? Pt.walk_cut & 0xffu : 0u, cut_round = cut ? (Pt.walk_cut >> 8) & 0xffu : 0u;
					intersect_grids<true>(objs, Pt.n_objects, grids, lds_masks, scr, want && waiting, ro, rd, part_t, part_obj, part_sub, Pt.debug_flags, Pt.debug_counters,
					                      cut_lanes, carry, &carried, cut_round, Pt.grid_mask);
					waiting = carried;
				} else {
					intersect_grids<false>(objs, Pt.n_objects, grids, lds_masks, scr, want && waiting, ro, rd, part_t, part_obj, part_sub, Pt.debug_flags, Pt.debug_counters, 0u, nullptr, nullptr, 0u,
					                       Pt.grid_mask);
					waiting = false;
				}
			}
			RMD_TSTAMP(tt_walk)
			complete = want && !waiting;
			t = part_t, oi = part_obj, sub = part_sub;
		} else {
			oi = scene_intersect_wave<false>(objs, Pt.n_objects, grids, lds_masks, scr, want, ro, rd, t, sub, Pt.axis_pairs, Pt.debug_flags, Pt.debug_counters, false, Pt.visit_mask);
			complete = want;
		}
	}

#if RMD_DIAG
	if (tstamp && lane == 0) {
		atomicAdd(&P.debug_counters[0], __builtin_amdgcn_s_memtime() - tt_begin), atomicAdd(&P.debug_counters[1], tt_b);
		atomicAdd(&P.debug_counters[2], tt_simple), atomicAdd(&P.debug_counters[3], tt_walk), atomicAdd(&P.debug_counters[4], tt_class);
	}
#endif
#undef RMD_TSTAMP
	if constexpr (to_buffer && !GRID) finish_sample_range(P, tile, wt, P.split_k, false, lane, out);
	if (writes && !to_buffer && !acc_in_memory) {
		out[out_index + 0] = acc.x;
		out[out_index + 1] = acc.y;
		out[out_index + 2] = acc.z;
		if constexpr (MOM && !acc_in_memory) out_sq[out_index + 0] = acc_sq.x, out_sq[out_index + 1] = acc_sq.y, out_sq[out_index + 2] = acc_sq.z;
	}
}

constexpr int kSortObjPrio = 1;
struct alignas(16) HitStack {
	double frag[3][kSortSlots], T[3][kSortSlots];
	uint32_t state[kSortSlots];
	uint32_t lobe_bits[kSortSlots];
	uint32_t item[kSortSlots];
};
static_assert(kSortSlots >= 72u && kSortSlots <= 512u && kSortSlots % 8u == 0u, "a generation trip needs room for 64 more hits");
static_assert(sizeof(HitStack) == kSortPoolBytes, "launch.hpp: kSortPoolBytes");
using SortPool = HitStack;

RMD_DEV void item_candidates(KernargWords kernarg_params, WaveTile tile, const DevObject *__restrict__ objs, const DevObject *lobjs, uint32_t *sets) {
	const uint32_t lane = threadIdx.x & 63u;
	KernargWords src = kernarg_params;
	asm volatile("" : "+s"(src));
	unsigned long long w[sizeof(RenderParams) / 8];
#pragma unroll
	for (unsigned i = 0; i < sizeof(RenderParams) / 8; i++) w[i] = src[i];
	RenderParams P;
	__builtin_memcpy(&P, w, sizeof(P));
	unsigned long long visit = P.visit_mask;
	uint32_t pairs = P.axis_pairs;
	if (P.primary_cull != 0u) {
		CullCamera cc;
		cc.pos[0] = P.cam_pos[0], cc.pos[1] = P.cam_pos[1], cc.pos[2] = P.cam_pos[2];
		cc.width = P.width, cc.height = P.height, cc.aspect = P.aspect, cc.tan_half_fov = P.tan_half_fov;
		const TileCone cone = primary_tile_cone(cc, tile.x0, tile.y0, tile.w, tile.h);
		const DevObject &o = lobjs[lane < P.n_objects ? lane : 0u];
		const double centre[3] = {o.origin[0], o.origin[1], o.origin[2]};
		const bool cleared = lane < P.n_objects && o.geometry_kind == 1u && primary_sphere_cleared(cone, cc, centre, o.radius);
		visit &= ~__ballot(cleared);
		const AxisWalls *walls = reinterpret_cast<const AxisWalls *>(objs + P.n_objects);
		const AxisWalls w3[3] = {walls[0], walls[1], walls[2]};
		pairs = primary_pairs_kept(cone, cc, w3, P.axis_pairs);
	}
	if (lane == 0u) sets[0] = pairs, sets[1] = (uint32_t)visit, sets[2] = (uint32_t)(visit >> 32);
	__builtin_amdgcn_fence(__ATOMIC_RELEASE, "wavefront");
	__builtin_amdgcn_wave_barrier();
	__builtin_amdgcn_fence(__ATOMIC_ACQUIRE, "wavefront");
}
#define RMD_UNDEF3(v) RMD_UNDEF(v.x) RMD_UNDEF(v.y) RMD_UNDEF(v.z)
template <bool MOM = false>
RMD_DEV void render_wave_sorted(const RenderParams &P, KernargWords kernarg_params, const DevObject *__restrict__ objs, const DevGrid *__restrict__ grids,
                                const void *__restrict__ work, double *__restrict__ out, const DevObject *lobjs, unsigned char *wave_lds, uint32_t work_item,
                                double *__restrict__ out_sq = nullptr) {
	const uint32_t lane = threadIdx.x & 63u;
	HitStack &stack = *reinterpret_cast<HitStack *>(wave_lds);
	WalkScratch *no_scratch = nullptr;
	const WorkItem wi = work_list_item(work_item, P.n_work, P.n_whole, P.split_k, P.sample_count);
	const uint32_t wt = wi.tile;
	const bool have = wt < P.n_work;
	const WaveTile tile = reinterpret_cast<const WaveTile *>(work)[have ? wt : 0];
	const uint32_t pool_first = wi.first, pool_items = wi.count * 64u;
	if (P.bounce_limit == 0u) return;
	const V3 cam_pos = ld3(P.cam_pos);

	uint32_t *item_sets = reinterpret_cast<uint32_t *>(wave_lds + sizeof(HitStack)) + 1;
	item_candidates(kernarg_params, tile, objs, lobjs, item_sets);

	uint32_t n_d = 0, n_g = 0, next_item = 0;
	unsigned long long trips_left = lobe_trip_bound(pool_items, kTripBoundPerPair);
#if RMD_DIAG
	if (P.debug_flags & 32u) trips_left = 1ull;
#endif
	for (;;) {
		KernargWords src = kernarg_params;
		asm volatile("" : "+s"(src));
		unsigned long long w[sizeof(RenderParams) / 8];
#pragma unroll
		for (unsigned i = 0; i < sizeof(RenderParams) / 8; i++) w[i] = src[i];
		RenderParams Pt;
		__builtin_memcpy(&Pt, w, sizeof(Pt));

		if (RMD_UNLIKELY(trips_left-- == 0ull)) {
			report_fault(Pt, kFaultSortedTripLoop, work_item);
			n_d = 0u, n_g = 0u, next_item = pool_items;
		}
		const LobeTrip trip = lobe_trip_rule(n_d, n_g, next_item < pool_items, kSortSlots);
		if (trip.kind == kTripDone) break;
		const bool shade_trip = trip.kind != kTripGenerate;
		bool active;
		uint32_t item = 0, depth = 1;
		Rng rng;
		rng.block = 0u, rng.lobe_bits = 0u;
		V3 ro, rd, T;
		RMD_UNDEF3(ro) RMD_UNDEF3(rd) RMD_UNDEF3(T)
		bool failed = false;
		unsigned long long turns = Pt.visit_mask;
		uint32_t pairs = Pt.axis_pairs;
		if (shade_trip) {
			const bool lobe_d = trip.kind == kTripShadeDiffuse;
			const uint32_t n = trip.lanes;
			active = lane < n;
			const uint32_t e = lobe_pop_first(lobe_d, n_d, n_g, n, kSortSlots) + (active ? lane : 0u);
			if (lobe_d) n_d -= n;
			else n_g -= n;
#if RMD_DIAG
			if ((Pt.debug_flags & 8u) && Pt.debug_counters && lane == 0u)
				atomicAdd(&Pt.debug_counters[lobe_d ? 37 : 39], 1ull), atomicAdd(&Pt.debug_counters[lobe_d ? 38 : 40], (unsigned long long)n);
#endif
			const uint32_t st = stack.state[e];
			item = stack.item[e];
			const uint32_t lb = stack.lobe_bits[e];
			rng.block = st >> 16, rng.lobe_bits = lb & 0x3FFFFFu;
			depth = lb >> 24;
			const DevObject &o = lobjs[st & 0xFFFFu];
			T = mk(stack.T[0][e], stack.T[1][e], stack.T[2][e]);
			const V3 frag = mk(stack.frag[0][e], stack.frag[1][e], stack.frag[2][e]);
			V3 normal;
			if (o.geometry_kind == 0u) normal = ld3(o.normal);
			else normal = normalize(frag - ld3(o.origin));
			const uint32_t x = tile.x0 + (item & 7u), y = tile.y0 + ((item >> 3) & 7u);
			rng.pixel = y * Pt.W + x, rng.sample = Pt.sample_begin + pool_first + (item >> 6);
			{
				if (lobe_d) shade_lobe<true>(Pt, normal, frag, ld3(o.color), o.roughness, o.metalness, cam_pos, rng, ro, rd, T);
				else shade_lobe<false>(Pt, normal, frag, ld3(o.color), o.roughness, o.metalness, cam_pos, rng, ro, rd, T);
				depth++;
				const bool black = Pt.end_black_paths != 0u && T.x == 0.0 && T.y == 0.0 && T.z == 0.0;
				failed = active && (depth > Pt.bounce_limit || black);
			}
		} else {
			item = next_item + lane;
			next_item += 64u;
			active = item < pool_items && (item & 7u) < tile.w && ((item >> 3) & 7u) < tile.h;
			const uint32_t x = tile.x0 + (item & 7u), y = tile.y0 + ((item >> 3) & 7u);
			rng.pixel = y * Pt.W + x, rng.sample = Pt.sample_begin + pool_first + (item >> 6);
			T = mk(1.0, 1.0, 1.0);
			{
				double u0, u1;
				rng.next2(Pt.key0, Pt.key1, u0, u1);
				primary_ray(Pt, x, y, u0, u1, ro, rd);
				if (Pt.use_dof) failed = active && !thin_lens_from_pinhole(Pt, ro, rd, rng, ro, rd);
			}
			pairs = (uint32_t)__builtin_amdgcn_readfirstlane((int)item_sets[0]);
			turns = (unsigned long long)(uint32_t)__builtin_amdgcn_readfirstlane((int)item_sets[1]) | (unsigned long long)(uint32_t)__builtin_amdgcn_readfirstlane((int)item_sets[2]) << 32;
		}
		const bool want = active && !failed;
		double t = 0.0;
		uint32_t sub = 0;
		__builtin_amdgcn_s_setprio(kSortObjPrio);
		const int oi = scene_intersect_wave<false>(objs, Pt.n_objects, grids, nullptr, *no_scratch, want, ro, rd, t, sub, pairs, 0u, nullptr, false, turns);
		__builtin_amdgcn_s_setprio(0);
#if RMD_DIAG
		if ((Pt.debug_flags & 512u) && (Pt.debug_flags & 8u) && Pt.debug_counters && !shade_trip) {
			double t_full = 0.0;
			uint32_t sub_full = 0;
			const int oi_full = scene_intersect_wave<false>(objs, Pt.n_objects, grids, nullptr, *no_scratch, want, ro, rd, t_full, sub_full, Pt.axis_pairs, 0u, nullptr, false, Pt.visit_mask);
			const bool differs = want && (oi_full != oi || __builtin_bit_cast(unsigned long long, t_full) != __builtin_bit_cast(unsigned long long, t));
			unsigned long long wrong = 0ull;
			const unsigned long long dropped = Pt.visit_mask & ~turns;
			for (unsigned long long m = dropped; m != 0ull; m &= m - 1ull) {
				const DevObject &o = objs[__builtin_ctzll(m)];
				double ts;
				wrong += (unsigned long long)__popcll(__ballot(want && sphere_test_flat(ld3(o.origin), o.radius, ro, rd, ts)));
			}
			const unsigned long long dm = __ballot(differs), wm = __ballot(want);
			if (lane == 0u) {
				atomicAdd(&Pt.debug_counters[32], (unsigned long long)__popcll(wm)), atomicAdd(&Pt.debug_counters[33], wrong);
				atomicAdd(&Pt.debug_counters[34], (unsigned long long)__popcll(dm)), atomicAdd(&Pt.debug_counters[35], (unsigned long long)__popcll(dropped));
				atomicAdd(&Pt.debug_counters[36], pairs != Pt.axis_pairs ? 1ull : 0ull);
			}
		}
#endif
		bool terminal = failed, park = false, emitted = false;
		bool park_d = false;
		V3 frag;
		RMD_UNDEF3(frag)
		if (want) {
			if (oi < 0) {
				terminal = true;
			} else {
				const DevObject &o = lobjs[oi];
				frag = ro + rd * t;
				if (o.material_kind == 2u) {
					emitted = true;
					terminal = true;
				} else {
					const bool black_bounce = Pt.end_black_paths != 0u && (o.flags & kObjBlackDiffuse) != 0u && rng.lobe_bits < (1u << 21);
					park = true;
					if ((depth == Pt.bounce_limit && Pt.shade_last_depth == 0u) || black_bounce) {
						V3 normal;
						if (o.geometry_kind == 0u) normal = ld3(o.normal);
						else normal = normalize(frag - ld3(o.origin));
						const double probe_sum = ((normal.x + normal.y) + normal.z) + ((frag.x + frag.y) + frag.z);
						const bool finite_inputs = __builtin_fabs(probe_sum) < __builtin_inf();
						if (finite_inputs) terminal = true, park = false;
					}
					double prob_d;
					park_d = bounce_is_diffuse(lobe_uniform(rng.lobe_bits), o.metalness, prob_d);
				}
			}
		}
		if (active && terminal) {
			V3 L = mk(0.0, 0.0, 0.0);
			if (emitted) L = ld3(lobjs[oi].color);
			L = hadamard(T, L);
			RMD_GLOBAL double *dst = (RMD_GLOBAL double *)Pt.sample_buf + (((size_t)wt * Pt.sample_count + pool_first + (item >> 6)) * 64u + (item & 63u)) * kSampleStride;
			store_sample(dst, L);
		}
		{
			const unsigned long long pm_d = __ballot(park && park_d), pm_g = __ballot(park && !park_d);
			const uint32_t rank_d = __builtin_amdgcn_mbcnt_hi((uint32_t)(pm_d >> 32), __builtin_amdgcn_mbcnt_lo((uint32_t)pm_d, 0u));
			const uint32_t rank_g = __builtin_amdgcn_mbcnt_hi((uint32_t)(pm_g >> 32), __builtin_amdgcn_mbcnt_lo((uint32_t)pm_g, 0u));
			const uint32_t e = lobe_push_entry(park_d, n_d, n_g, park_d ? rank_d : rank_g, kSortSlots);
			if (park) {
				stack.frag[0][e] = frag.x, stack.frag[1][e] = frag.y, stack.frag[2][e] = frag.z;
				stack.T[0][e] = T.x, stack.T[1][e] = T.y, stack.T[2][e] = T.z;
				stack.state[e] = (uint32_t)oi | (rng.block << 16);
				stack.lobe_bits[e] = rng.lobe_bits | (depth << 24), stack.item[e] = item;
			}
			n_d += (uint32_t)__popcll(pm_d), n_g += (uint32_t)__popcll(pm_g);
#if RMD_DIAG
			if ((Pt.debug_flags & 8u) && Pt.debug_counters && lane == 0u)
				atomicAdd(&Pt.debug_counters[41], (unsigned long long)__popcll(pm_d)), atomicAdd(&Pt.debug_counters[42], (unsigned long long)__popcll(pm_g));
#endif
			__builtin_amdgcn_fence(__ATOMIC_RELEASE, "wavefront");
			__builtin_amdgcn_wave_barrier();
			__builtin_amdgcn_fence(__ATOMIC_ACQUIRE, "wavefront");
		}
	}
	finish_sample_range<MOM>(P, tile, wt, P.split_k, work_item < P.n_whole, lane, out, out_sq);
}

struct PathQueues {
	RMD_GLOBAL double *hit_d;
	RMD_GLOBAL double *ray_d;
	RMD_GLOBAL uint32_t *hit_w;
	RMD_GLOBAL uint32_t *ray_w;
	uint32_t cap;
};
constexpr uint32_t kRayCarried = 1u << 23;
__host__ __device__ inline size_t path_queue_bytes(uint32_t cap) { return (size_t)cap * (9u * 8u + 13u * 8u + 4u * 4u + 9u * 4u); }
RMD_DEV uint32_t sample_of_sector(const RenderParams &P, uint32_t sector) {
	const uint32_t a = sector >> 6, q = (uint32_t)__umul64hi((unsigned long long)a, P.sample_magic);
	return P.sample_begin + (P.sample_magic != 0ull ? a - q * P.sample_count : 0u);
}
constexpr uint32_t kQueuedTripBoundPerPath = 2u * RMD_MAX_BOUNCE_LIMIT_DEV + 4u;
constexpr size_t kQueuedSideBytes = 64u * (3u * sizeof(double) + 4u * sizeof(uint32_t));
constexpr size_t kQueuedDiagBytes = RMD_DIAG ? 24u * sizeof(unsigned long long) : 0u;
__host__ __device__ inline size_t queued_wave_lds_bytes() { return sizeof(WalkScratch) + sizeof(WalkCarry) + kQueuedSideBytes + kQueuedDiagBytes + kWaveHeadBytes; }

template <class T>
RMD_DEV T qld(const RMD_GLOBAL T *p) {
	return *p;
}
template <class T, class U>
RMD_DEV void qst(RMD_GLOBAL T *p, U v) {
	*p = (T)v;
}
RMD_DEV void render_wave_queued(const RenderParams &P, KernargWords kernarg_params, const DevObject *__restrict__ objs, const DevGrid *__restrict__ grids,
                                const void *__restrict__ work, const DevObject *lobjs, const uint32_t *lds_masks, unsigned char *wave_lds, uint32_t first_item) {
	const uint32_t lane = threadIdx.x & 63u;
	WalkScratch &scr = *reinterpret_cast<WalkScratch *>(wave_lds);
	WalkCarry *carry = reinterpret_cast<WalkCarry *>(wave_lds + sizeof(WalkScratch));
	double *side_d = reinterpret_cast<double *>(wave_lds + sizeof(WalkScratch) + sizeof(WalkCarry)) + lane;
	uint32_t *side_w = reinterpret_cast<uint32_t *>(wave_lds + sizeof(WalkScratch) + sizeof(WalkCarry) + 192u * sizeof(double)) + lane;
	if (P.bounce_limit == 0u) return;
#if RMD_DIAG
	volatile unsigned long long *qacc = reinterpret_cast<volatile unsigned long long *>(wave_lds + sizeof(WalkScratch) + sizeof(WalkCarry) + kQueuedSideBytes);
	if (lane < 24u) qacc[lane] = 0ull;
#endif
	PathQueues q;
	{
		constexpr uint32_t cap = kQueuePaths;
		const uint32_t wave_index = (uint32_t)__builtin_amdgcn_readfirstlane((int)(blockIdx.x * (blockDim.x >> 6) + (threadIdx.x >> 6)));
		RMD_GLOBAL unsigned char *base = (RMD_GLOBAL unsigned char *)P.queue_buf + (size_t)wave_index * path_queue_bytes(cap);
		q.cap = cap;
		q.hit_d = (RMD_GLOBAL double *)base;
		q.ray_d = q.hit_d + (size_t)9u * cap;
		q.hit_w = (RMD_GLOBAL uint32_t *)(q.ray_d + (size_t)13u * cap);
		q.ray_w = q.hit_w + (size_t)4u * cap;
	}
	enum { kGen = 0, kShade = 1, kWalk = 2 };

	uint32_t wt = 0, pool_first = 0, pool_items = 0, next_item = 0;
	WaveTile tile = {};
	auto take_item = [&](const RenderParams &Q, uint32_t drawn) {
		wt = drawn / Q.split_k;
		const uint32_t part = drawn - wt * Q.split_k;
		tile = reinterpret_cast<const WaveTile *>(work)[wt];
		const uint32_t per_part = (Q.sample_count + Q.split_k - 1u) / Q.split_k;
		const uint32_t s_lo = part * per_part < Q.sample_count ? part * per_part : Q.sample_count;
		const uint32_t s_hi = s_lo + per_part < Q.sample_count ? s_lo + per_part : Q.sample_count;
		pool_first = s_lo, pool_items = (s_hi - s_lo) * 64u, next_item = 0u;
	};
	if (first_item / P.split_k < P.n_work) take_item(P, first_item);
	uint32_t n_hit = 0, n_ray = 0;
	const unsigned long long trips_per_path = kQueuedTripBoundPerPath + (unsigned long long)RMD_MAX_BOUNCE_LIMIT_DEV * P.walk_steps_bound;
	unsigned long long trips_left = ((unsigned long long)pool_items + q.cap) * trips_per_path + 64ull;
#if RMD_DIAG
	if (P.debug_flags & 32u) trips_left = 1ull;
#endif
	bool rheld = false;
	double *stash_a = reinterpret_cast<double *>(wave_lds) + lane;
	int32_t *stash_oi = reinterpret_cast<int32_t *>(wave_lds + 256u * sizeof(double)) + lane;
	double *stash_b = reinterpret_cast<double *>(wave_lds + sizeof(WalkScratch)) + lane;
	static_assert(sizeof(WalkScratch) >= 256u * sizeof(double) + 64u * sizeof(int32_t) && sizeof(WalkCarry) >= 192u * sizeof(double), "a held ray's columns");
	bool held = false;
	V3 h_frag, h_normal, h_T;
	RMD_UNDEF3(h_frag) RMD_UNDEF3(h_normal) RMD_UNDEF3(h_T)
	uint32_t h_st = 0, h_lb = 0, h_px = 0, h_sector = 0;
	for (;;) {
		KernargWords src = kernarg_params;
// ... 260 lines not shown
		{
			const unsigned long long pm = __ballot(park);
			const uint32_t n_park = (uint32_t)__popcll(pm);
			const bool hold = n_park != 0u && !rhold && n_ray < 64u && n_hit + n_park >= 64u;
			h_frag = frag, h_normal = normal, h_T = T;
			h_st = (uint32_t)oi | (rng_block << 16), h_lb = lobe_bits | (depth << 24), h_px = pxw, h_sector = sector;
			held = hold && park;
#if RMD_DIAG
			if ((Pt.debug_flags & 8u) && Pt.debug_counters && lane == 0 && n_park != 0u) atomicAdd(&Pt.debug_counters[hold ? 21 : 20], (unsigned long long)n_park);
#endif
			if (pm != 0ull && !hold) {
				constexpr uint32_t cap = kQueuePaths;
				const uint32_t e = n_hit + __builtin_amdgcn_mbcnt_hi((uint32_t)(pm >> 32), __builtin_amdgcn_mbcnt_lo((uint32_t)pm, 0u));
				if (park) {
					qst(&q.hit_d[e], frag.x), qst(&q.hit_d[cap + e], frag.y), qst(&q.hit_d[2u * cap + e], frag.z);
					qst(&q.hit_d[3u * cap + e], normal.x), qst(&q.hit_d[4u * cap + e], normal.y), qst(&q.hit_d[5u * cap + e], normal.z);
					qst(&q.hit_d[6u * cap + e], T.x), qst(&q.hit_d[7u * cap + e], T.y), qst(&q.hit_d[8u * cap + e], T.z);
					qst(&q.hit_w[e], h_st);
					qst(&q.hit_w[cap + e], h_lb);
					qst(&q.hit_w[2u * cap + e], pxw), qst(&q.hit_w[3u * cap + e], sector);
				}
				n_hit += n_park;
			}
		}
		RMD_QSTAMP(6u)
#if RMD_DIAG
		if (qstamp && lane == 0u) qacc[kind * 8u + 7u] += 1ull;
#endif
	}
#undef RMD_QSTAMP
#undef RMD_QSTAMP_FETCH
#if RMD_DIAG
	if ((P.debug_flags & 16u) && P.debug_counters && lane < 24u) atomicAdd(&P.debug_counters[lane], qacc[lane]);
#endif
}

template <int MODE, bool GRID>
constexpr bool kSortedTrips = MODE == kModeTilesBuffered && !GRID;
template <int MODE, bool GRID>
constexpr bool kChainItems = MODE == kModeTilesBuffered && GRID;
template <int MODE, bool GRID>
constexpr bool kPathQueues = MODE == kModeTilesBuffered && GRID;
template <int MODE, bool GRID, bool QUEUED = false>
__host__ __device__ inline size_t wave_lds_of(uint32_t n_grids) { return QUEUED ? queued_wave_lds_bytes() : kSortedTrips<MODE, GRID> ? kWaveHeadBytes + sizeof(SortPool) : wave_lds_bytes(n_grids); }
template <int MODE, bool GRID>
constexpr uint32_t kPersistWaves = kSortedTrips<MODE, GRID> ? kSortedWavesPerWg : GRID ? kGridPersistWavesPerWg : kPersistWavesPerWg;
template <int MODE, bool GRID, bool PERSIST>
constexpr int kWgThreads = PERSIST ? 64 * (kPersistWaves<MODE, GRID>) : GRID ? 64 * kGridWavesPerWg : 64;
template <int MODE, bool GRID, bool PERSIST>
constexpr int kMinWavesPerSimd = GRID ? kGridMinWaves : (kSortedTrips<MODE, GRID>) ? kSortedWavesPerWg / 4 : (PERSIST ? 4 : kNoGridMinWaves);
template <int MODE, bool GRID>
constexpr bool kMomentsInKernel = MODE == kModeTiles || (MODE == kModeTilesBuffered && !GRID);
template <int MODE, bool GRID, bool PERSIST, bool CHAIN, bool QUEUED, bool MOM>
RMD_DEV void render_kernel_body(const RenderParams &P, const DevObject *__restrict__ objs, const DevGrid *__restrict__ grids, const void *__restrict__ work,
                                double *__restrict__ out, int32_t *__restrict__ path_obj, uint32_t *__restrict__ path_sub, double *__restrict__ out_sq) {
	static_assert(!MOM || (kMomentsInKernel<MODE, GRID> && !CHAIN && !QUEUED), "the squares are added where the samples are");
	extern __shared__ __align__(16) unsigned char smem[];
	const KernargWords kernarg_params = (KernargWords)__builtin_amdgcn_kernarg_segment_ptr();
	DevObject *lobjs = reinterpret_cast<DevObject *>(smem);
	uint32_t *lmasks = reinterpret_cast<uint32_t *>(smem + (size_t)P.n_objects * sizeof(DevObject));
	const uint32_t tid = threadIdx.x, wave = tid >> 6, waves_per_wg = blockDim.x >> 6;
	unsigned char *wave_lds = smem + (size_t)P.n_objects * sizeof(DevObject) + (size_t)((P.mask_words_total + 3u) & ~3u) * 4u +
	                          (size_t)wave * wave_lds_of<MODE, GRID, QUEUED>(P.n_grids);
	[[maybe_unused]] unsigned char *wave_head = wave_lds + wave_lds_of<MODE, GRID, QUEUED>(P.n_grids) - kWaveHeadBytes;
	{
		const double *src = reinterpret_cast<const double *>(objs);
		double *dst = reinterpret_cast<double *>(lobjs);
		for (uint32_t i = tid; i < P.n_objects * 16u; i += blockDim.x) dst[i] = src[i];
		for (uint32_t gi = 0; gi < P.n_grids; gi++) {
			const DevGrid &g = grids[gi];
			if (g.mask_lds_word == 0xFFFFFFFFu) continue;
			for (uint32_t i = tid; i < g.mask_n_words; i += blockDim.x) lmasks[g.mask_lds_word + i] = as_global(g.mask_words)[i];
		}
	}
	__syncthreads();
	const uint32_t *lds_masks = P.mask_words_total ? lmasks : nullptr;
	if constexpr (PERSIST) {
		static_assert(MODE != kModeList, "list launches are not persistent");
		const uint32_t n_items = kSortedTrips<MODE, GRID> ? work_list_items(P.n_work, P.n_whole, P.split_k) : P.n_work * (MODE == kModeTilesBuffered ? P.split_k : 1u);
		volatile uint32_t *last_draw = reinterpret_cast<volatile uint32_t *>(wave_head);
		if ((tid & 63u) == 0u) *last_draw = 0u;
		for (;;) {
			uint32_t item = 0, floor = 0;
			if ((tid & 63u) == 0u) {
				item = atomicAdd(P.work_counter, 1u);
				floor = *last_draw;
				*last_draw = item + 1u;
#if RMD_DIAG
				if ((P.debug_flags & 128u) && floor != 0u) floor = 0xFFFFFFFFu;
#endif
			}
			item = (uint32_t)__builtin_amdgcn_readfirstlane((int)item);
			if (item >= n_items) break;
			floor = (uint32_t)__builtin_amdgcn_readfirstlane((int)floor);
			if (RMD_UNLIKELY(item < floor)) {
				report_fault(P, kFaultWorkLoop, item);
				break;
			}
			if constexpr (QUEUED) render_wave_queued(P, kernarg_params, objs, grids, work, lobjs, lds_masks, wave_lds, item);
			else if constexpr (kSortedTrips<MODE, GRID>) render_wave_sorted<MOM>(P, kernarg_params, objs, grids, work, out, lobjs, wave_lds, item, out_sq);
			else render_wave<MODE, GRID, CHAIN, MOM>(P, kernarg_params, objs, grids, work, out, path_obj, path_sub, lobjs, lds_masks, wave_lds, item, out_sq);
		}
	} else {
		const uint32_t unit = work_item_of_block(blockIdx.x, gridDim.x) * waves_per_wg + wave;
		if constexpr (kSortedTrips<MODE, GRID>) render_wave_sorted<MOM>(P, kernarg_params, objs, grids, work, out, lobjs, wave_lds, unit, out_sq);
		else render_wave<MODE, GRID, false, MOM>(P, kernarg_params, objs, grids, work, out, path_obj, path_sub, lobjs, lds_masks, wave_lds, MODE == kModeList ? unit * 64u : unit, out_sq);
	}
}
template <int MODE, bool GRID, bool PERSIST, bool CHAIN = false, bool QUEUED = false>
__global__ __launch_bounds__((kWgThreads<MODE, GRID, PERSIST>), (kMinWavesPerSimd<MODE, GRID, PERSIST>)) void render_kernel(
    RenderParams P, const DevObject *__restrict__ objs, const DevGrid *__restrict__ grids, const void *__restrict__ work, double *__restrict__ out,
    int32_t *__restrict__ path_obj, uint32_t *__restrict__ path_sub) {
	render_kernel_body<MODE, GRID, PERSIST, CHAIN, QUEUED, false>(P, objs, grids, work, out, path_obj, path_sub, nullptr);
}
template <int MODE, bool GRID, bool PERSIST>
__global__ __launch_bounds__((kWgThreads<MODE, GRID, PERSIST>), (kMinWavesPerSimd<MODE, GRID, PERSIST>)) void render_kernel_moments(
    RenderParams P, const DevObject *__restrict__ objs, const DevGrid *__restrict__ grids, const void *__restrict__ work, double *__restrict__ out,
    int32_t *__restrict__ path_obj, uint32_t *__restrict__ path_sub, double *__restrict__ out_sq) {
	render_kernel_body<MODE, GRID, PERSIST, false, false, true>(P, objs, grids, work, out, path_obj, path_sub, out_sq);
}

template <int MODE, bool GRID>
inline LaunchPlan plan_launch(uint32_t n_objects, uint32_t mask_words_total, bool queues, bool persist, bool chain_items, bool moments, uint32_t n_waves,
                              uint32_t n_cus) {
	LaunchPlan L;
	const size_t fixed = (size_t)n_objects * sizeof(DevObject) + (size_t)((mask_words_total + 3u) & ~3u) * 4u;
	const size_t wave = wave_lds_of<MODE, GRID>(GRID ? 1u : 0u);
	L.moments = kMomentsInKernel<MODE, GRID> && moments ? 1u : 0u;
	if (MODE != kModeList && persist) {
		const bool queued = kPathQueues<MODE, GRID> && queues;
		const size_t pwave = queued ? wave_lds_of<MODE, GRID, true>(1u) : wave;
		uint32_t pw = kPersistWaves<MODE, GRID>;
		while (pw > 4u && fixed + pw * pwave > kLdsBudgetBytes) pw--;
		if (fixed + pw * pwave <= kLdsBudgetBytes) {
			const uint32_t wgs = (n_waves + pw - 1u) / pw;
			L.persistent = 1u, L.waves_per_wg = pw, L.wave_lds = pwave, L.lds = fixed + pw * pwave, L.workgroups = wgs < n_cus ? wgs : n_cus;
			L.queued = queued ? 1u : 0u;
			L.chained = kChainItems<MODE, GRID> && chain_items && !queued ? 1u : 0u;
			return L;
		}
	}
	uint32_t w = GRID ? kGridWavesPerWg : 1u;
	while (w > 1u && fixed + w * wave > kLdsBudgetBytes) w--;
	L.waves_per_wg = w, L.wave_lds = wave, L.lds = fixed + w * wave, L.workgroups = (n_waves + w - 1u) / w;
	return L;
}

template <int MODE, bool GRID>
inline hipError_t launch_render(hipStream_t stream, const RenderParams &P, const DevObject *objs, const DevGrid *grids, const void *work,
                                uint32_t n_waves, double *out, int32_t *path_obj, uint32_t *path_sub, uint32_t n_cus = 0, LaunchShape *shape = nullptr,
                                double *out_sq = nullptr) {
	const LaunchPlan L = plan_launch<MODE, GRID>(P.n_objects, P.mask_words_total, P.queue_buf != nullptr, n_cus != 0u && P.work_counter != nullptr,
	                                             P.chain_items != 0u, out_sq != nullptr, n_waves, n_cus);
	if (L.lds > kLdsBudgetBytes) return hipErrorInvalidConfiguration;
	const void *fn = nullptr;
	if constexpr (MODE != kModeList) {
		if (L.persistent) {
			fn = L.queued    ? reinterpret_cast<const void *>(&render_kernel<MODE, GRID, true, false, (kPathQueues<MODE, GRID>)>)
			     : L.chained ? reinterpret_cast<const void *>(&render_kernel<MODE, GRID, true, (kChainItems<MODE, GRID>)>)
			                 : reinterpret_cast<const void *>(&render_kernel<MODE, GRID, true>);
			if constexpr (kMomentsInKernel<MODE, GRID>) {
				if (L.moments) fn = reinterpret_cast<const void *>(&render_kernel_moments<MODE, GRID, true>);
			}
		}
	}
	if (!fn) {
// ... 34 lines not shown
```

raymond_amd/probe.py:

```python
import ctypes as C
import os

import numpy as np

from . import abi
from . import lib as _lib

_vp = C.c_void_p
_sz = C.c_size_t
_P = C.POINTER
_SIGS = {
    "rmd_probe_philox4x32_10": [_vp, _sz, _vp, _vp, _vp],
    "rmd_probe_block_uniforms": [_vp, C.c_uint64, _sz, _vp, _vp, _vp, _vp],
    "rmd_probe_sphere_intersect": [_vp, _sz, _vp, _vp, _vp, _vp],
    "rmd_probe_sphere_normal": [_vp, _sz, _vp, _vp, _vp, _vp],
    "rmd_probe_plane_intersect": [_vp, _sz, _vp, _vp, _vp, _vp],
    "rmd_probe_aabb_intersect": [_vp, _sz, _vp, _vp, _vp, _vp],
    "rmd_probe_triangle_intersect": [_vp, _sz, _vp, _vp, _vp, _vp],
    "rmd_probe_triangle_normal": [_vp, _sz, _vp, _vp, _vp, _vp, _vp],
    "rmd_probe_onb": [_vp, _sz, _vp, _vp, _vp],
    "rmd_probe_cosine_hemisphere": [_vp, _sz, _vp, _vp, _vp, _vp],
    "rmd_probe_importance_sample_ggx": [_vp, _sz, _vp, _vp, _vp, _vp, _vp],
    "rmd_probe_ggx_distribution": [_vp, _sz, _vp, _vp, _vp, _vp],
    "rmd_probe_geometry_smith": [_vp, _sz, _vp, _vp, _vp, _vp, _vp],
    "rmd_probe_fresnel_schlick": [_vp, _sz, _vp, _vp, _vp],
    "rmd_probe_primary_ray": [_vp, _sz, _P(abi.Camera), _vp, _vp, _vp],
    "rmd_probe_elementary": [_vp, _sz, _vp, _vp, _vp, _vp, _vp, _vp],
    "rmd_probe_scene_intersect": [_vp, _vp, _sz, _vp, _vp, _vp, _vp],
    "rmd_probe_grid_intersect": [_vp, _vp, C.c_uint32, _sz, _vp, _vp, _vp, _vp],
    "rmd_probe_grid_intersect_deep": [_vp, _vp, C.c_uint32, _sz, _vp, C.c_uint32, C.c_uint32, C.c_uint32, _vp, _vp, _vp],
    "rmd_probe_trace_samples": [_vp, _vp, _P(abi.Camera), _P(abi.Settings), _sz, _vp, _vp, _vp, _vp, _vp],
    "rmd_probe_triangle_sphere": [_sz, _vp, _vp],
    "rmd_probe_pretest_pairs": [_vp, _sz, _vp, _vp, _vp, _vp, _vp, _vp],
    "rmd_probe_primary_candidates": [_P(abi.Camera), _P(abi.Settings), _P(abi.Object), C.c_uint32, C.c_uint32, C.c_int64, _sz, _vp, _vp, _vp],
    "rmd_probe_launch_plan": [C.c_uint32, C.c_uint32, _sz, _vp, _vp],
    "rmd_probe_launch_sizes": [C.c_uint32, C.c_uint32, _vp],
    "rmd_probe_work_plan": [_vp, _sz, _vp, _vp],
    "rmd_probe_work_items": [C.c_uint32, C.c_uint32, C.c_uint32, C.c_uint32, C.c_uint32, _sz, _vp, _P(C.c_uint32)],
    "rmd_probe_scene_layout": [_vp, _P(C.c_uint32), _P(C.c_uint32), _P(C.c_uint32)],
    "rmd_probe_scene_plan": [_vp, _vp, _sz, _vp],
    "rmd_probe_denoise_scratch": [C.c_uint32] * 6 + [C.c_uint64, _vp, _P(C.c_uint64)],
    "rmd_probe_feature_slope": [_vp, _vp, C.c_uint32, C.c_uint32, C.c_double, _vp],
    "rmd_probe_atrous_region_slope_planes": [_vp, C.c_uint32, C.c_uint32, _vp],
    "rmd_probe_denoise_scratch_slope": [C.c_uint32] * 7 + [C.c_uint64, _vp, _P(C.c_uint64)],
    "rmd_probe_denoise_tile": [C.c_uint32, C.c_uint32, _vp],
}
PATH_STRIDE = 17
_ready = False


PROBE_LIB_PATH = os.path.join(os.path.dirname(_lib.LIB_PATH), "libraymond_hip_probe.so")
_probe_lib = None


def _L():
    global _ready, _probe_lib
    if not _ready:
        _lib.load()
        if not os.path.exists(PROBE_LIB_PATH):
            raise ImportError("raymond_amd.probe: %s is missing — build it with `python -c 'import __graft_entry__ as g; g.build()'`" % PROBE_LIB_PATH)
        _probe_lib = C.CDLL(PROBE_LIB_PATH)
        for name, args in _SIGS.items():
            fn = getattr(_probe_lib, name)
            fn.restype, fn.argtypes = C.c_int32, args
        _ready = True
    return _probe_lib


def _p(a):
    return a.ctypes.data_as(C.c_void_p)


def _f(a, w=None):
    a = np.ascontiguousarray(a, dtype=np.float64)
    return a if w is None else a.reshape(-1, w)


def hit_t(ctx, name, shape, rays):
    L = _L()
    rays = _f(rays, 6)
    shape = _f(shape).reshape(rays.shape[0], -1)
    n = rays.shape[0]
    hit = np.zeros(n, dtype=np.int32)
    t = np.zeros(n)
    ctx.check(getattr(L, "rmd_probe_%s_intersect" % name)(ctx.handle, n, _p(shape), _p(rays), _p(hit), _p(t)))
    return hit, t


def call(ctx, name, n, ins, outs):
    L = _L()
    ins = [_f(a) for a in ins]
    res = [np.zeros((n, w)) for w in outs]
    ctx.check(getattr(L, "rmd_probe_" + name)(ctx.handle, n, *[_p(a) for a in ins], *[_p(a) for a in res]))
    return res


def philox(ctx, ctr, key):
    L = _L()
    ctr = np.ascontiguousarray(ctr, dtype=np.uint32).reshape(-1, 4)
    key = np.ascontiguousarray(key, dtype=np.uint32).reshape(-1, 2)
    out = np.zeros_like(ctr)
    ctx.check(L.rmd_probe_philox4x32_10(ctx.handle, ctr.shape[0], _p(ctr), _p(key), _p(out)))
    return out


def block_uniforms(ctx, seed, pixel, sample, block):
    L = _L()
    pixel, sample, block = (np.ascontiguousarray(a, dtype=np.uint32) for a in (pixel, sample, block))
    out = np.zeros((pixel.shape[0], 5))
    ctx.check(L.rmd_probe_block_uniforms(ctx.handle, seed, pixel.shape[0], _p(pixel), _p(sample), _p(block), _p(out)))
    return out


def elementary(ctx, x):
    L = _L()
    x = _f(x).ravel()
    s, si, co, ro, ir = (np.zeros_like(x) for _ in range(5))
# ... 14 lines not shown
def scene_intersect(ctx, dscene, rays):
    L = _L()
    rays = _f(rays, 6)
    n = rays.shape[0]
    obj = np.zeros(n, dtype=np.int32)
    t = np.zeros(n)
    sub = np.zeros(n, dtype=np.uint32)
    ctx.check(L.rmd_probe_scene_intersect(ctx.handle, dscene.handle, n, _p(rays), _p(obj), _p(t), _p(sub)))
    return obj, t, sub


def grid_intersect(ctx, dscene, g, rays):
    L = _L()
    rays = _f(rays, 6)
    n = rays.shape[0]
    hit = np.zeros(n, dtype=np.int32)
    t = np.zeros(n)
    tri = np.zeros(n, dtype=np.uint32)
    ctx.check(L.rmd_probe_grid_intersect(ctx.handle, dscene.handle, g, n, _p(rays), _p(hit), _p(t), _p(tri)))
    return hit, t, tri


def grid_intersect_deep(ctx, dscene, g, rays, cut_lanes=0, cut_round=0, rays_per_wave=64):
    L = _L()
    rays = _f(rays, 6)
    n = rays.shape[0]
    hit = np.zeros(n, dtype=np.int32)
    t = np.zeros(n)
    tri = np.zeros(n, dtype=np.uint32)
    ctx.check(L.rmd_probe_grid_intersect_deep(ctx.handle, dscene.handle, g, n, _p(rays), cut_lanes, cut_round, rays_per_wave, _p(hit), _p(t), _p(tri)))
    return hit, t, tri


def trace_samples(ctx, dscene, cam, settings, xy, samples, paths=False):
    L = _L()
    xy = np.ascontiguousarray(xy, dtype=np.uint32).reshape(-1, 2)
    samples = np.ascontiguousarray(samples, dtype=np.uint32)
    n = xy.shape[0]
    rgb = np.zeros((n, 3))
    po = np.full((n, PATH_STRIDE), -2, dtype=np.int32) if paths else None
    ps = np.zeros((n, PATH_STRIDE), dtype=np.uint32) if paths else None
    c, s = cam.pod(), settings.pod()
    ctx.check(
        L.rmd_probe_trace_samples(ctx.handle, dscene.handle, C.byref(c), C.byref(s), n, _p(xy), _p(samples), _p(rgb),
                                  _p(po) if paths else None, _p(ps) if paths else None)
    )
    return (rgb, po, ps) if paths else rgb


def triangle_sphere(pos9):
    from . import abi as _abi

    L = _L()
    pos9 = _f(pos9, 9)
    out = np.zeros((pos9.shape[0], 5))
    st = L.rmd_probe_triangle_sphere(pos9.shape[0], _p(pos9), _p(out))
    if st != _abi.RMD_OK:
        raise RuntimeError("rmd_probe_triangle_sphere: status %d" % st)
    return out[:, :3], out[:, 3], out[:, 4]


def pretest_pairs(ctx, sphere5, pos9, ray6):
    L = _L()
    sphere5, pos9, ray6 = _f(sphere5, 5), _f(pos9, 9), _f(ray6, 6)
    n = pos9.shape[0]
    passed, hit, t = np.zeros(n, dtype=np.int32), np.zeros(n, dtype=np.int32), np.zeros(n)
    ctx.check(L.rmd_probe_pretest_pairs(ctx.handle, n, _p(sphere5), _p(pos9), _p(ray6), _p(passed), _p(hit), _p(t)))
    return passed.astype(bool), hit.astype(bool), t


def primary_candidates(cam, settings, scene, tiles, axis_pairs_tunable=0):
    L = _L()
    objs, n, _descs, ng, keep = scene.flatten()
    tiles = np.ascontiguousarray(tiles, dtype=np.uint32).reshape(-1, 4)
    launch, out = np.zeros(3, dtype=np.uint64), np.zeros((tiles.shape[0], 2), dtype=np.uint64)
    c, s = cam.pod(), settings.pod()
    st = L.rmd_probe_primary_candidates(C.byref(c), C.byref(s), objs, n, ng, int(axis_pairs_tunable), tiles.shape[0], _p(tiles), _p(launch), _p(out))
    del keep
    if st != abi.RMD_OK:
        raise RuntimeError("rmd_probe_primary_candidates: status %d" % st)
    return int(launch[0]), int(launch[1]), bool(launch[2]), out[:, 0].copy(), out[:, 1].astype(np.uint32)


MODE_TILES, MODE_TILES_BUFFERED, MODE_LIST = 0, 1, 2
PLAN_QUEUES, PLAN_PERSIST, PLAN_CHAIN, PLAN_MOMENTS = 1, 2, 4, 8
PLAN_FIELDS = ("persistent", "queued", "chained", "moments", "waves_per_wg", "workgroups", "wave_lds", "lds")
SIZE_FIELDS = ("budget", "object", "wave", "queued_wave", "persist_waves", "grid_waves", "sort_pool", "mask_budget")


def _host_check(st, name):
    if st != abi.RMD_OK:
        raise RuntimeError("%s: status %d" % (name, st))


def launch_plan(mode, grid, n_objects, mask_words_total, flags, n_waves, n_cus):
    L = _L()
    cols = np.broadcast_arrays(*(np.asarray(a, dtype=np.int64) for a in (n_objects, mask_words_total, flags, n_waves, n_cus)))
    inp = np.ascontiguousarray(np.stack([c.ravel() for c in cols], axis=1).astype(np.uint32))
    out = np.zeros((inp.shape[0], 8), dtype=np.uint64)
    _host_check(L.rmd_probe_launch_plan(mode, int(grid), inp.shape[0], _p(inp), _p(out)), "rmd_probe_launch_plan")
    return {k: out[:, i].astype(np.int64).reshape(cols[0].shape) for i, k in enumerate(PLAN_FIELDS)}


def launch_sizes(mode, grid):
    L = _L()
    out = np.zeros(8, dtype=np.uint64)
    _host_check(L.rmd_probe_launch_sizes(mode, int(grid), _p(out)), "rmd_probe_launch_sizes")
    return {k: int(v) for k, v in zip(SIZE_FIELDS, out)}


def work_plan(wave_slots, n_tiles, sample_count, k_uniform, ctx=None, pass_samples=0):
    L = _L()
    if ctx is not None:
        wave_slots = pass_samples
    cols = np.broadcast_arrays(*(np.asarray(a, dtype=np.int64) for a in (wave_slots, n_tiles, sample_count, k_uniform)))
    inp = np.ascontiguousarray(np.stack([c.ravel() for c in cols], axis=1).astype(np.uint32))
    out = np.zeros((inp.shape[0], 3), dtype=np.uint32)
    _host_check(L.rmd_probe_work_plan(ctx.handle if ctx is not None else None, inp.shape[0], _p(inp), _p(out)), "rmd_probe_work_plan")
    return tuple(out[:, i].astype(np.int64).reshape(cols[0].shape) for i in range(3))


WORK_ITEM_FIELDS = ("tile", "first", "count", "parts", "whole")


def work_items(n_tiles, n_whole, k_tail, sample_count, extra=0):
    L = _L()
    n_items = C.c_uint32()
    _host_check(L.rmd_probe_work_items(n_tiles, n_whole, k_tail, sample_count, 0, 0, None, C.byref(n_items)), "rmd_probe_work_items")
    out = np.zeros((n_items.value + extra, 5), dtype=np.uint32)
    _host_check(L.rmd_probe_work_items(n_tiles, n_whole, k_tail, sample_count, 0, out.shape[0], _p(out), C.byref(n_items)), "rmd_probe_work_items")
    return out.astype(np.int64), n_items.value


def scene_layout(dscene):
    L = _L()
    n, g, m = C.c_uint32(), C.c_uint32(), C.c_uint32()
    _host_check(L.rmd_probe_scene_layout(dscene.handle, C.byref(n), C.byref(g), C.byref(m)), "rmd_probe_scene_layout")
    return n.value, g.value, m.value


SCENE_PLAN_FIELDS = ("n_grid_objects", "regular", "walk_steps_bound", "axis_pairs", "visit_mask", "grid_mask", "n_grids")


def scene_plan(dscene):
    L = _L()
    out = np.zeros(8, dtype=np.uint64)
    _host_check(L.rmd_probe_scene_plan(dscene.handle, _p(out), 0, None), "rmd_probe_scene_plan")
    n = int(out[6])
    per_grid = np.zeros((max(n, 1), 2), dtype=np.uint32)
    _host_check(L.rmd_probe_scene_plan(dscene.handle, _p(out), n, _p(per_grid)), "rmd_probe_scene_plan")
    plan = {k: int(v) for k, v in zip(SCENE_PLAN_FIELDS, out)}
    plan["mask_shift"], plan["mask_bits"] = [int(v) for v in per_grid[:n, 0]], [int(v) for v in per_grid[:n, 1]]
    return plan


def feature_slope(ctx, f, fvalid, slope):
    L = _L()
    H, W = fvalid.shape
    planes = np.ascontiguousarray(np.moveaxis(np.asarray(f, dtype=np.float64), -1, 0)).copy()
    planes[0][~np.asarray(fvalid, dtype=bool)] = np.nan
    out = np.zeros_like(planes)
    ctx.check(L.rmd_probe_feature_slope(ctx.handle, _p(planes), W, H, float(slope), _p(out)))
    return np.moveaxis(out, 0, -1).copy()


def atrous_region_slope_planes(ctx, width, height):
# ... 31 lines not shown
```

Baseline: 26690.

## Classify wave tiles by the lone wall they see and shortcut emitter/black tiles

```diff
diff --git a/include/raymond_hip_probe.h b/include/raymond_hip_probe.h
--- a/include/raymond_hip_probe.h
+++ b/include/raymond_hip_probe.h
@@ -41,6 +41,8 @@
 rmd_status rmd_probe_triangle_sphere(size_t n, const double *pos9, double *out5);
 rmd_status rmd_probe_primary_candidates(const rmd_camera *cam, const rmd_settings *settings, const rmd_object *objects, uint32_t n_objects, uint32_t n_grids,
                                         int64_t axis_pairs_tunable, size_t n_tiles, const uint32_t *tiles4, uint64_t *launch3, uint64_t *out2);
+rmd_status rmd_probe_tile_classes(const rmd_camera *cam, const rmd_settings *settings, const rmd_object *objects, uint32_t n_objects, uint32_t n_grids,
+                                  int64_t axis_pairs_tunable, size_t n_tiles, const uint32_t *tiles4, uint32_t *launch1, int32_t *out2);
 rmd_status rmd_probe_launch_plan(uint32_t mode, uint32_t grid, size_t n, const uint32_t *in5, uint64_t *out8);
 rmd_status rmd_probe_launch_sizes(uint32_t mode, uint32_t grid, uint64_t *out8);
 rmd_status rmd_probe_work_plan(const rmd_context *ctx, size_t n, const uint32_t *in4, uint32_t *out3);
diff --git a/raymond_amd/csrc/api.cpp b/raymond_amd/csrc/api.cpp
--- a/raymond_amd/csrc/api.cpp
+++ b/raymond_amd/csrc/api.cpp
@@ -193,9 +193,9 @@
 	return P.use_dof == 0u && cull_camera_ok(c);
 }
 
-static bool camera_on_a_plane(const rmd_scene *scene, const rmd_camera *cam) {
-	for (size_t i = 0; i + 6 <= scene->planes.size(); i += 6) {
-		const double *o = &scene->planes[i], *n = o + 3;
+bool camera_on_a_plane(const std::vector<double> &planes, const rmd_camera *cam) {
+	for (size_t i = 0; i + 6 <= planes.size(); i += 6) {
+		const double *o = &planes[i], *n = o + 3;
 		double num = 0.0, scale = 0.0;
 		for (int a = 0; a < 3; a++) num += (o[a] - cam->position[a]) * -n[a], scale += (std::fabs(o[a]) + std::fabs(cam->position[a])) * std::fabs(n[a]);
 		if (!(std::fabs(num) > 1e-9 * scale)) return true;
@@ -223,12 +223,12 @@
 	P.mask_words_total = scene ? scene->mask_words_total : 0;
 	P.key0 = (uint32_t)st->seed, P.key1 = (uint32_t)(st->seed >> 32);
 	P.use_dof = ((st->flags & RMD_RENDER_DOF) && cam->aperture_radius > 0.0) ? 1u : 0u;
-	const bool on_plane = scene && camera_on_a_plane(scene, cam);
-	P.end_black_paths = (st->flags & RMD_RENDER_TRACE_BLACK_PATHS) ? 0u : ((st->flags & RMD_RENDER_END_BLACK_PATHS) || !scene || (scene->n_grids == 0u && scene->regular && !on_plane)) ? 1u : 0u;
+	const bool on_plane = scene && rmd::camera_on_a_plane(scene->planes, cam);
+	P.end_black_paths = rmd::end_black_paths_rule(st->flags, scene != nullptr, scene ? scene->n_grids : 0u, scene ? scene->regular : false, on_plane) ? 1u : 0u;
 	P.shade_last_depth = (scene && (!scene->regular || on_plane)) ? 1u : 0u;
 	P.axis_pairs = scene ? scene->axis_pairs : 0u;
 	P.visit_mask = scene ? scene->visit_mask : ~0ull, P.grid_mask = scene ? scene->grid_mask : ~0ull;
-	P.primary_cull = (scene && scene->primary_cull && rmd::primary_cull_allowed(P)) ? 1u : 0u;
+	P.primary_cull = (scene && rmd::primary_cull_allowed(P)) ? (scene->primary_cull & (P.end_black_paths != 0u ? 3u : 1u)) : 0u;
 	P.fault = ctx ? ctx->d_fault : nullptr;
 	P.walk_batch = rmd::kWalkBatchDefault;
 	if (ctx && ctx->tunable[RMD_TUNE_WALK_BATCH] > 0) P.walk_batch = (uint32_t)ctx->tunable[RMD_TUNE_WALK_BATCH];
@@ -474,7 +474,7 @@
 	sc->visit_mask = derived.visit_mask, sc->grid_mask = derived.grid_mask;
 	for (uint32_t i = 0; i < n_objects; i++)
 		if (objects[i].geometry_kind == RMD_GEOM_PLANE) sc->planes.insert(sc->planes.end(), objects[i].origin, objects[i].origin + 3), sc->planes.insert(sc->planes.end(), objects[i].normal, objects[i].normal + 3);
-	sc->primary_cull = regular && n_grids == 0u && ctx->tunable[RMD_TUNE_AXIS_PAIRS] == 0;
+	sc->primary_cull = rmd::primary_cull_bits(regular, n_grids, ctx->tunable[RMD_TUNE_AXIS_PAIRS]);
 	for (uint32_t i = 0; i < n_objects; i++) sc->n_grid_objects += objects[i].geometry_kind == RMD_GEOM_GRID ? 1u : 0u;
 	auto upload = [&](const void *src, size_t bytes, void **dst) -> hipError_t {
 		*dst = nullptr;
@@ -694,8 +694,8 @@
 	rmd::RenderParams P = rmd::make_params(ctx, scene, camera, settings);
 	P.n_work = ctx->n_wave_tiles;
 	if (P.debug_flags & 24u) {
-		RMD_HIP(ctx, ctx->debug_counters.grow(48 * sizeof(unsigned long long)));
-		RMD_HIP(ctx, hipMemsetAsync(ctx->debug_counters.as<void>(), 0, 48 * sizeof(unsigned long long), ctx->stream));
+		RMD_HIP(ctx, ctx->debug_counters.grow(64 * sizeof(unsigned long long)));
+		RMD_HIP(ctx, hipMemsetAsync(ctx->debug_counters.as<void>(), 0, 64 * sizeof(unsigned long long), ctx->stream));
 		P.debug_counters = ctx->debug_counters.as<unsigned long long>();
 	}
 	bool buffered = false;
@@ -785,7 +785,7 @@
 	RMD_HIP(ctx, hipEventRecord(ctx->ev_stop, ctx->stream));
 	ctx->timed = true;
 	if (P.debug_flags & 24u) {
-		unsigned long long h[48];
+		unsigned long long h[64];
 		RMD_HIP(ctx, hipMemcpyAsync(h, ctx->debug_counters.as<void>(), sizeof(h), hipMemcpyDeviceToHost, ctx->stream));
 		RMD_HIP(ctx, hipStreamSynchronize(ctx->stream));
 		if ((P.debug_flags & 16u) && ctx->last_launch.queued) {
@@ -809,6 +809,9 @@
 		if ((P.debug_flags & 16u) == 0u && ctx->last_launch.buffered && scene->n_grids == 0u)
 			std::fprintf(stderr, "[rmd debug] lobe trips: diffuse trips=%llu diffuse hits shaded=%llu ggx trips=%llu ggx hits shaded=%llu | hits parked: diffuse=%llu ggx=%llu\n", h[37], h[38], h[39],
 			             h[40], h[41], h[42]);
+		if ((P.debug_flags & 16u) == 0u && ctx->last_launch.buffered && scene->n_grids == 0u)
+			std::fprintf(stderr, "[rmd debug] tile classes: general items=%llu emitter items=%llu black items=%llu | black rounds=%llu cut short=%llu samples ended in pass A=%llu survivors=%llu | samples checked against their full path=%llu that are not what the class says (must be 0)=%llu rays that hit another object than the wall (must be 0)=%llu\n",
+			             h[48], h[49], h[50], h[52], h[54], h[51], h[53], h[55], h[56], h[57]);
 		if ((P.debug_flags & 16u) == 0u && ctx->last_launch.queued)
 			std::fprintf(stderr, "[rmd debug] path queues: rays pushed=%llu (of them walks put aside=%llu) rays held in their lanes=%llu hits pushed=%llu hits held in their lanes=%llu\n", h[19], h[22], h[23], h[20], h[21]);
 	}
diff --git a/raymond_amd/csrc/internal.hpp b/raymond_amd/csrc/internal.hpp
--- a/raymond_amd/csrc/internal.hpp
+++ b/raymond_amd/csrc/internal.hpp
@@ -110,7 +110,7 @@
 	uint32_t axis_pairs = 0;
 	unsigned long long visit_mask = ~0ull, grid_mask = ~0ull;
 	uint32_t walk_steps_bound = 0;
-	bool primary_cull = false;
+	uint32_t primary_cull = 0;
 	bool regular = true;
 	std::vector<double> planes;
 	rmd::DevObject *d_objects = nullptr;
@@ -211,6 +211,14 @@
 rmd_status check_fault(rmd_context *ctx);
 RenderParams make_params(const rmd_context *ctx, const rmd_scene *scene, const rmd_camera *cam, const rmd_settings *st);
 bool primary_cull_allowed(const RenderParams &P);
+inline uint32_t primary_cull_bits(bool regular, uint32_t n_grids, int64_t axis_pairs_tunable) {
+	if (!regular || n_grids != 0u) return 0u;
+	return axis_pairs_tunable == 0 ? 3u : axis_pairs_tunable == 3 ? 1u : 0u;
+}
+inline bool end_black_paths_rule(uint32_t flags, bool has_scene, uint32_t n_grids, bool regular, bool on_plane) {
+	return (flags & RMD_RENDER_TRACE_BLACK_PATHS) ? false : ((flags & RMD_RENDER_END_BLACK_PATHS) || !has_scene || (n_grids == 0u && regular && !on_plane));
+}
+bool camera_on_a_plane(const std::vector<double> &planes, const rmd_camera *cam);
 WorkPlan plan_work_list(uint32_t wave_slots, uint32_t n_tiles, uint32_t sample_count, uint32_t k_uniform, uint32_t min_samples = kTailMinSamples,
                         uint32_t tail_x2 = kTailTilesPerSlotX2, uint32_t tail_parts = kTailParts, uint32_t n_tail_forced = 0u);
 WorkPlan context_work_plan(const rmd_context *ctx, bool has_grid, uint32_t n_tiles, uint32_t sample_count, uint32_t pass_samples);
diff --git a/raymond_amd/csrc/primary_candidates.hpp b/raymond_amd/csrc/primary_candidates.hpp
--- a/raymond_amd/csrc/primary_candidates.hpp
+++ b/raymond_amd/csrc/primary_candidates.hpp
@@ -78,36 +78,69 @@
 	return in_front && D > r + margin && K <= 1e150;
 }
 
-RMD_HD uint32_t primary_pairs_kept(const TileCone &T, const CullCamera &c, const AxisWalls walls[3], uint32_t axis_pairs) {
-	if (!T.ok) return axis_pairs;
+RMD_HD bool primary_pair_alone(const TileCone &T, const CullCamera &c, const AxisWalls walls[3], uint32_t axis_pairs, int &k_alone, bool &faces_minus) {
+	if (!T.ok) return false;
 	double s_lo[3], s_hi[3];
-	bool paired[3];
+	bool paired[3], minus[3];
+#pragma unroll
 	for (int k = 0; k < 3; k++) {
 		paired[k] = ((axis_pairs >> (10 * k)) & 1023u) != 0u;
-		s_lo[k] = 0.0, s_hi[k] = -1.0;
+		s_lo[k] = 0.0, s_hi[k] = -1.0, minus[k] = false;
 		if (!paired[k]) continue;
 		const double num_plus = c.pos[k] - walls[k].o_plus, num_minus = walls[k].o_minus - c.pos[k];
-		if (!(num_plus > 0.0 && num_minus > 0.0)) return axis_pairs;
+		if (!(num_plus > 0.0 && num_minus > 0.0)) return false;
 		const double lo = k < 2 ? T.lo[k] : 1.0, hi = k < 2 ? T.hi[k] : 1.0;
 		double nearest = 1e300;
 		if (hi > 0.0) nearest = cull_min(nearest, num_minus / hi);
 		if (lo < 0.0) nearest = cull_min(nearest, num_plus / -lo);
 		s_lo[k] = nearest;
-		if (!(s_lo[k] > 0.0)) return axis_pairs;
+		if (!(s_lo[k] > 0.0)) return false;
 		const bool pos = lo > 0.0, neg = hi < 0.0;
 		if (pos || neg) {
 			const double u_lo = pos ? lo : -hi;
-			if (u_lo > kCullFacing * T.u_max) s_hi[k] = (pos ? num_minus : num_plus) / u_lo;
+			if (u_lo > kCullFacing * T.u_max) s_hi[k] = (pos ? num_minus : num_plus) / u_lo, minus[k] = pos;
 		}
 	}
+	bool found = false;
+#pragma unroll
 	for (int k = 0; k < 3; k++) {
-		if (!paired[k] || !(s_hi[k] > 0.0)) continue;
-		bool alone = true;
+		bool alone = paired[k] && s_hi[k] > 0.0 && !found;
+#pragma unroll
 		for (int j = 0; j < 3; j++)
 			if (j != k && paired[j]) alone = alone && s_hi[k] * (1.0 + kCullPairMargin) < s_lo[j];
-		if (alone) return axis_pairs & (1023u << (10 * k));
+		if (alone) found = true, k_alone = k, faces_minus = minus[k];
 	}
-	return axis_pairs;
+	return found;
+}
+RMD_HD uint32_t primary_pairs_kept(const TileCone &T, const CullCamera &c, const AxisWalls walls[3], uint32_t axis_pairs) {
+	int k = 0;
+	bool faces_minus = false;
+	return primary_pair_alone(T, c, walls, axis_pairs, k, faces_minus) ? axis_pairs & (1023u << (10 * k)) : axis_pairs;
+}
+
+enum : uint32_t { kTileGeneral = 0u, kTileEmitter = 1u, kTileBlack = 2u };
+constexpr uint32_t kTileClassShift = 30u;
+RMD_HD int primary_one_wall(bool alone, bool faces_minus, const AxisWalls &pair, unsigned long long visit, uint32_t n_objects) {
+	return (alone && visit == 0ull && n_objects - 1u < 64u) ?
+	       (int)(faces_minus ? pair.idx_minus : pair.idx_plus) : -1;
+}
+RMD_HD uint32_t primary_wall_class(uint32_t material_kind, uint32_t flags, double metalness);
+RMD_HD uint32_t primary_tile_class(bool alone, int k_alone, bool faces_minus, const AxisWalls *walls, unsigned long long visit, uint32_t n_objects, const DevObject *objs,
+                                   uint32_t &wall);
+RMD_HD uint32_t primary_wall_class(uint32_t material_kind, uint32_t flags, double metalness) {
+	if (material_kind == 2u) return kTileEmitter;
+	const double prob_d = 0.5 + metalness * (0.0 - 0.5);
+	return ((flags & kObjBlackDiffuse) != 0u && prob_d == 0.5) ? kTileBlack : kTileGeneral;
+}
+RMD_HD uint32_t primary_tile_class(bool alone, int k_alone, bool faces_minus, const AxisWalls *walls, unsigned long long visit, uint32_t n_objects, const DevObject *objs,
+                                   uint32_t &wall) {
+	wall = 0u;
+	const int w = primary_one_wall(alone, faces_minus, walls[alone ? k_alone : 0], visit, n_objects);
+	if (w < 0) return kTileGeneral;
+	const DevObject &o = objs[w];
+	const uint32_t cls = primary_wall_class(o.material_kind, o.flags, o.metalness);
+	if (cls != kTileGeneral) wall = (uint32_t)w;
+	return cls;
 }
 
 }
diff --git a/raymond_amd/csrc/probe.cpp b/raymond_amd/csrc/probe.cpp
--- a/raymond_amd/csrc/probe.cpp
+++ b/raymond_amd/csrc/probe.cpp
@@ -247,7 +247,7 @@
 		rmd::SceneObjects sc;
 		if (rmd_status s = rmd::derive_scene_objects(nullptr, objects, n_objects, n_grids, axis_pairs_tunable, sc)) return s;
 		const rmd::RenderParams P = rmd::make_params(nullptr, nullptr, cam, settings);
-		const bool on = sc.regular && n_grids == 0u && axis_pairs_tunable == 0 && rmd::primary_cull_allowed(P);
+		const bool on = (rmd::primary_cull_bits(sc.regular, n_grids, axis_pairs_tunable) & 1u) != 0u && rmd::primary_cull_allowed(P);
 		launch3[0] = sc.visit_mask, launch3[1] = sc.axis_pairs, launch3[2] = on ? 1u : 0u;
 		rmd::CullCamera cc;
 		for (int a = 0; a < 3; a++) cc.pos[a] = P.cam_pos[a];
@@ -269,6 +269,42 @@
 	});
 }
 
+rmd_status rmd_probe_tile_classes(const rmd_camera *cam, const rmd_settings *settings, const rmd_object *objects, uint32_t n_objects, uint32_t n_grids,
+                                  int64_t axis_pairs_tunable, size_t n_tiles, const uint32_t *tiles4, uint32_t *launch1, int32_t *out2) {
+	if (!cam || !settings || (n_objects && !objects) || !launch1 || (n_tiles != 0 && (!tiles4 || !out2))) return rmd::fail(nullptr, RMD_ERR_INVALID_ARGUMENT, "probe: bad argument");
+	return rmd::guarded(nullptr, "rmd_probe_tile_classes", [&]() -> rmd_status {
+		rmd::SceneObjects sc;
+		if (rmd_status s = rmd::derive_scene_objects(nullptr, objects, n_objects, n_grids, axis_pairs_tunable, sc)) return s;
+		const rmd::RenderParams P = rmd::make_params(nullptr, nullptr, cam, settings);
+		std::vector<double> planes;
+		for (uint32_t i = 0; i < n_objects; i++)
+			if (objects[i].geometry_kind == RMD_GEOM_PLANE) planes.insert(planes.end(), objects[i].origin, objects[i].origin + 3), planes.insert(planes.end(), objects[i].normal, objects[i].normal + 3);
+		const bool end_black = rmd::end_black_paths_rule(settings->flags, true, n_grids, sc.regular, rmd::camera_on_a_plane(planes, cam));
+		const bool on = rmd::primary_cull_bits(sc.regular, n_grids, axis_pairs_tunable) == 3u && rmd::primary_cull_allowed(P) && end_black;
+		launch1[0] = on ? 1u : 0u;
+		rmd::CullCamera cc;
+		for (int a = 0; a < 3; a++) cc.pos[a] = P.cam_pos[a];
+		cc.width = P.width, cc.height = P.height, cc.aspect = P.aspect, cc.tan_half_fov = P.tan_half_fov;
+		for (size_t i = 0; i < n_tiles; i++) {
+			const uint32_t *t = tiles4 + i * 4;
+			out2[i * 2] = (int32_t)rmd::kTileGeneral, out2[i * 2 + 1] = -1;
+			if (!on) continue;
+			if (t[2] == 0u || t[2] > 8u || t[3] == 0u || t[3] > 8u || t[0] > 65535u || t[1] > 65535u) return rmd::fail(nullptr, RMD_ERR_INVALID_ARGUMENT, "probe: a wave tile is 1..8 pixels a side");
+			const rmd::TileCone cone = rmd::primary_tile_cone(cc, t[0], t[1], t[2], t[3]);
+			uint64_t visit = sc.visit_mask;
+			for (uint32_t j = 0; j < n_objects && j < 64u; j++)
+				if (sc.objs[j].geometry_kind == 1u && rmd::primary_sphere_cleared(cone, cc, sc.objs[j].origin, sc.objs[j].radius)) visit &= ~(1ull << j);
+			int k_alone = 0;
+			bool faces_minus = false;
+			const bool alone = rmd::primary_pair_alone(cone, cc, sc.walls, sc.axis_pairs, k_alone, faces_minus);
+			uint32_t wall = 0u;
+			const uint32_t cls = rmd::primary_tile_class(alone, k_alone, faces_minus, sc.walls, visit, n_objects, sc.objs.data(), wall);
+			out2[i * 2] = (int32_t)cls, out2[i * 2 + 1] = cls == rmd::kTileGeneral ? -1 : (int32_t)wall;
+		}
+		return RMD_OK;
+	});
+}
+
 rmd_status rmd_probe_launch_plan(uint32_t mode, uint32_t grid, size_t n, const uint32_t *in5, uint64_t *out8) {
 	if (mode > 2u || grid > 1u || (n != 0 && (!in5 || !out8))) return rmd::fail(nullptr, RMD_ERR_INVALID_ARGUMENT, "probe: bad argument");
 	for (size_t i = 0; i < n; i++) {
diff --git a/raymond_amd/csrc/render_kernel.hpp b/raymond_amd/csrc/render_kernel.hpp
--- a/raymond_amd/csrc/render_kernel.hpp
+++ b/raymond_amd/csrc/render_kernel.hpp
@@ -6,6 +6,7 @@
 #include "launch.hpp"
 #include "lobe_trips.hpp"
 #include "primary_candidates.hpp"
+#include <type_traits>
 #include "scene_split.hpp"
 #include "work_list.hpp"
 
@@ -135,7 +136,9 @@
 		V3 sum = ld3(out + pix);
 		[[maybe_unused]] V3 sq = mk(0.0, 0.0, 0.0);
 		if constexpr (MOM) sq = ld3(out_sq + pix);
-		const RMD_GLOBAL double *src = (const RMD_GLOBAL double *)P.sample_buf + ((size_t)wt * P.sample_count * 64u + lane) * kSampleStride;
+		uint32_t sector = lane;
+		asm volatile("" : "+v"(sector));
+		const RMD_GLOBAL double *src = (const RMD_GLOBAL double *)P.sample_buf + ((size_t)wt * P.sample_count * 64u + sector) * kSampleStride;
 		constexpr uint32_t kInFlight = MOM ? 8u : 16u;
 		uint32_t k = 0;
 		for (; k + kInFlight <= P.sample_count; k += kInFlight) {
@@ -531,6 +534,11 @@
 }
 
 constexpr int kSortObjPrio = 1;
+#ifndef RMD_ROUND_PAIRS
+#define RMD_ROUND_PAIRS 128
+#endif
+constexpr uint32_t kRoundPairs = RMD_ROUND_PAIRS;
+static_assert(kRoundPairs > 64u && kRoundPairs <= 128u, "a round is two lane passes, the first a whole one");
 struct alignas(16) HitStack {
 	double frag[3][kSortSlots], T[3][kSortSlots];
 	uint32_t state[kSortSlots];
@@ -552,6 +560,7 @@
 	__builtin_memcpy(&P, w, sizeof(P));
 	unsigned long long visit = P.visit_mask;
 	uint32_t pairs = P.axis_pairs;
+	uint32_t cls = kTileGeneral, wall_obj = 0u;
 	if (P.primary_cull != 0u) {
 		CullCamera cc;
 		cc.pos[0] = P.cam_pos[0], cc.pos[1] = P.cam_pos[1], cc.pos[2] = P.cam_pos[2];
@@ -563,14 +572,44 @@
 		visit &= ~__ballot(cleared);
 		const AxisWalls *walls = reinterpret_cast<const AxisWalls *>(objs + P.n_objects);
 		const AxisWalls w3[3] = {walls[0], walls[1], walls[2]};
-		pairs = primary_pairs_kept(cone, cc, w3, P.axis_pairs);
-	}
-	if (lane == 0u) sets[0] = pairs, sets[1] = (uint32_t)visit, sets[2] = (uint32_t)(visit >> 32);
+		int k_alone = 0;
+		bool faces_minus = false;
+		const bool alone = primary_pair_alone(cone, cc, w3, P.axis_pairs, k_alone, faces_minus);
+		if (alone) pairs = P.axis_pairs & (1023u << (10 * k_alone));
+		if ((P.primary_cull & 2u) != 0u) {
+			cls = primary_tile_class(alone, k_alone, faces_minus, walls, visit, P.n_objects, lobjs, wall_obj);
+		}
+	}
+	if (lane == 0u) sets[0] = pairs | (cls << kTileClassShift), sets[1] = cls != kTileGeneral ? wall_obj : (uint32_t)visit, sets[2] = (uint32_t)(visit >> 32);
 	__builtin_amdgcn_fence(__ATOMIC_RELEASE, "wavefront");
 	__builtin_amdgcn_wave_barrier();
 	__builtin_amdgcn_fence(__ATOMIC_ACQUIRE, "wavefront");
 }
 #define RMD_UNDEF3(v) RMD_UNDEF(v.x) RMD_UNDEF(v.y) RMD_UNDEF(v.z)
+#if RMD_DIAG
+RMD_DEV void diag_check_black_zero(const RenderParams &Pt, const DevObject *__restrict__ objs, const DevObject *lobjs, const DevGrid *__restrict__ grids, const WaveTile &tile,
+                                   uint32_t item, bool ended, uint32_t w0, uint32_t w1, uint32_t w2, uint32_t w3, int wall) {
+	WalkScratch *no_scratch = nullptr;
+	double t_full = 0.0;
+	uint32_t sub_full = 0;
+	V3 fro, frd;
+	primary_ray(Pt, tile.x0 + (item & 7u), tile.y0 + ((item >> 3) & 7u), Rng::to_unit(w0, w1), Rng::to_unit(w2, w3), fro, frd);
+	const int oi_full = scene_intersect_wave<false>(objs, Pt.n_objects, grids, nullptr, *no_scratch, ended, fro, frd, t_full, sub_full, Pt.axis_pairs, 0u, nullptr, false, Pt.visit_mask);
+	bool zero = false;
+	if (oi_full >= 0) {
+		const DevObject &fo = lobjs[oi_full];
+		const V3 ffrag = fro + frd * t_full;
+		const double probe_sum = ((fo.normal[0] + fo.normal[1]) + fo.normal[2]) + ((ffrag.x + ffrag.y) + ffrag.z);
+		zero = fo.material_kind != 2u && fo.geometry_kind == 0u && (fo.flags & kObjBlackDiffuse) != 0u && Rng::spare22(w0, w2) < (1u << 21) && __builtin_fabs(probe_sum) < __builtin_inf();
+	}
+	const unsigned long long cm = __ballot(ended), bm = __ballot(ended && !zero), om = __ballot(ended && oi_full != wall);
+	if ((threadIdx.x & 63u) == 0u) {
+		atomicAdd(&Pt.debug_counters[57], (unsigned long long)__popcll(om));
+		atomicAdd(&Pt.debug_counters[55], (unsigned long long)__popcll(cm)), atomicAdd(&Pt.debug_counters[56], (unsigned long long)__popcll(bm));
+		atomicAdd(&Pt.debug_counters[32], (unsigned long long)__popcll(cm)), atomicAdd(&Pt.debug_counters[34], (unsigned long long)__popcll(bm));
+	}
+}
+#endif
 template <bool MOM = false>
 RMD_DEV void render_wave_sorted(const RenderParams &P, KernargWords kernarg_params, const DevObject *__restrict__ objs, const DevGrid *__restrict__ grids,
                                 const void *__restrict__ work, double *__restrict__ out, const DevObject *lobjs, unsigned char *wave_lds, uint32_t work_item,
@@ -590,10 +629,18 @@
 	item_candidates(kernarg_params, tile, objs, lobjs, item_sets);
 
 	uint32_t n_d = 0, n_g = 0, next_item = 0;
+#if RMD_DIAG
+	if ((P.debug_flags & 8u) && P.debug_counters && lane == 0u) {
+		const uint32_t cls = (uint32_t)__builtin_amdgcn_readfirstlane((int)item_sets[0]) >> kTileClassShift;
+		atomicAdd(&P.debug_counters[cls == kTileEmitter ? 49 : cls == kTileBlack ? 50 : 48], 1ull);
+	}
+#endif
 	unsigned long long trips_left = lobe_trip_bound(pool_items, kTripBoundPerPair);
 #if RMD_DIAG
 	if (P.debug_flags & 32u) trips_left = 1ull;
 #endif
+	auto trip_loop = [&](auto classed_item) {
+	constexpr bool CLASSED = decltype(classed_item)::value;
 	for (;;) {
 		KernargWords src = kernarg_params;
 		asm volatile("" : "+s"(src));
@@ -617,6 +664,9 @@
 		V3 ro, rd, T;
 		RMD_UNDEF3(ro) RMD_UNDEF3(rd) RMD_UNDEF3(T)
 		bool failed = false;
+#if RMD_DIAG
+		bool diag_emitter = false;
+#endif
 		unsigned long long turns = Pt.visit_mask;
 		uint32_t pairs = Pt.axis_pairs;
 		if (shade_trip) {
@@ -651,20 +701,100 @@
 				failed = active && (depth > Pt.bounce_limit || black);
 			}
 		} else {
+			const uint32_t head0 = (uint32_t)__builtin_amdgcn_readfirstlane((int)item_sets[0]);
+			const bool emitter_item = CLASSED && head0 >> kTileClassShift == kTileEmitter;
+			uint32_t w0, w1, w2, w3;
+			RMD_UNDEF(w0) RMD_UNDEF(w1) RMD_UNDEF(w2) RMD_UNDEF(w3)
 			item = next_item + lane;
 			next_item += 64u;
 			active = item < pool_items && (item & 7u) < tile.w && ((item >> 3) & 7u) < tile.h;
-			const uint32_t x = tile.x0 + (item & 7u), y = tile.y0 + ((item >> 3) & 7u);
-			rng.pixel = y * Pt.W + x, rng.sample = Pt.sample_begin + pool_first + (item >> 6);
+			rng.pixel = (tile.y0 + ((item >> 3) & 7u)) * Pt.W + tile.x0 + (item & 7u), rng.sample = Pt.sample_begin + pool_first + (item >> 6);
+			if (emitter_item) {
+				if (active) {
+					const V3 L = hadamard(mk(1.0, 1.0, 1.0), ld3(lobjs[(uint32_t)__builtin_amdgcn_readfirstlane((int)item_sets[1])].color));
+					RMD_GLOBAL double *dst = (RMD_GLOBAL double *)Pt.sample_buf + (((size_t)wt * Pt.sample_count + pool_first + (item >> 6)) * 64u + (item & 63u)) * kSampleStride;
+					store_sample(dst, L);
+				}
+#if RMD_DIAG
+				diag_emitter = active;
+#endif
+				active = false;
+			} else philox4x32_10(rng.pixel, rng.sample, 0u, 0u, Pt.key0, Pt.key1, w0, w1, w2, w3);
+			if (CLASSED && head0 >> kTileClassShift == kTileBlack) {
+				bool survivor = active && Rng::spare22(w0, w2) >= (1u << 21);
+				unsigned long long sm = __ballot(survivor);
+				uint32_t rank = __builtin_amdgcn_mbcnt_hi((uint32_t)(sm >> 32), __builtin_amdgcn_mbcnt_lo((uint32_t)sm, 0u));
+				if (active && !survivor) {
+					double zero = 0.0;
+					asm volatile("" : "+v"(zero));
+					RMD_GLOBAL double *dst = (RMD_GLOBAL double *)Pt.sample_buf + (((size_t)wt * Pt.sample_count + pool_first + (item >> 6)) * 64u + (item & 63u)) * kSampleStride;
+					store_sample(dst, mk(zero, zero, zero));
+				}
+				if (survivor) {
+					const uint32_t e = n_d + rank;
+					stack.item[e] = item, stack.state[e] = w0, stack.lobe_bits[e] = w1;
+					stack.frag[0][e] = __builtin_bit_cast(double, (unsigned long long)w2 | (unsigned long long)w3 << 32);
+				}
+				uint32_t staged = (uint32_t)__popcll(sm);
+#if RMD_DIAG
+				[[maybe_unused]] bool ended = active && !survivor;
+				if ((Pt.debug_flags & 8u) && Pt.debug_counters) {
+					const unsigned long long em = __ballot(ended);
+					if (lane == 0u) atomicAdd(&Pt.debug_counters[51], (unsigned long long)__popcll(em)), atomicAdd(&Pt.debug_counters[53], (unsigned long long)staged), atomicAdd(&Pt.debug_counters[52], 1ull);
+					if (Pt.debug_flags & 512u) diag_check_black_zero(Pt, objs, lobjs, grids, tile, item, ended, w0, w1, w2, w3, __builtin_amdgcn_readfirstlane((int)item_sets[1]));
+				}
+#endif
+				if (next_item < pool_items) {
+					item = next_item + lane;
+					active = lane < kRoundPairs - 64u && item < pool_items && (item & 7u) < tile.w && ((item >> 3) & 7u) < tile.h;
+					rng.pixel = (tile.y0 + ((item >> 3) & 7u)) * Pt.W + tile.x0 + (item & 7u), rng.sample = Pt.sample_begin + pool_first + (item >> 6);
+					philox4x32_10(rng.pixel, rng.sample, 0u, 0u, Pt.key0, Pt.key1, w0, w1, w2, w3);
+					survivor = active && Rng::spare22(w0, w2) >= (1u << 21);
+					sm = __ballot(survivor);
+					rank = staged + __builtin_amdgcn_mbcnt_hi((uint32_t)(sm >> 32), __builtin_amdgcn_mbcnt_lo((uint32_t)sm, 0u));
+					const unsigned long long over = __ballot(survivor && rank >= 64u);
+					const uint32_t used = over != 0ull ? (uint32_t)__builtin_ctzll(over) : kRoundPairs - 64u;
+					if (active && lane < used && !survivor) {
+						double zero = 0.0;
+						asm volatile("" : "+v"(zero));
+						RMD_GLOBAL double *dst = (RMD_GLOBAL double *)Pt.sample_buf + (((size_t)wt * Pt.sample_count + pool_first + (item >> 6)) * 64u + (item & 63u)) * kSampleStride;
+						store_sample(dst, mk(zero, zero, zero));
+					}
+					if (survivor && lane < used) {
+						const uint32_t e = n_d + rank;
+						stack.item[e] = item, stack.state[e] = w0, stack.lobe_bits[e] = w1;
+						stack.frag[0][e] = __builtin_bit_cast(double, (unsigned long long)w2 | (unsigned long long)w3 << 32);
+					}
+					const uint32_t more = (uint32_t)__popcll(__ballot(survivor && lane < used));
+					staged += more, next_item += used;
+#if RMD_DIAG
+					ended = active && lane < used && !survivor;
+					if ((Pt.debug_flags & 8u) && Pt.debug_counters) {
+						const unsigned long long em = __ballot(ended);
+						if (lane == 0u) atomicAdd(&Pt.debug_counters[51], (unsigned long long)__popcll(em)), atomicAdd(&Pt.debug_counters[53], (unsigned long long)more), atomicAdd(&Pt.debug_counters[54], over != 0ull ? 1ull : 0ull);
+						if (Pt.debug_flags & 512u) diag_check_black_zero(Pt, objs, lobjs, grids, tile, item, ended, w0, w1, w2, w3, __builtin_amdgcn_readfirstlane((int)item_sets[1]));
+					}
+#endif
+				}
+				__builtin_amdgcn_fence(__ATOMIC_RELEASE, "wavefront");
+				__builtin_amdgcn_wave_barrier();
+				__builtin_amdgcn_fence(__ATOMIC_ACQUIRE, "wavefront");
+				active = lane < staged;
+				const uint32_t e = n_d + (active ? lane : 0u);
+				const unsigned long long w23 = __builtin_bit_cast(unsigned long long, stack.frag[0][e]);
+				item = stack.item[e], w0 = stack.state[e], w1 = stack.lobe_bits[e], w2 = (uint32_t)w23, w3 = (uint32_t)(w23 >> 32);
+				rng.pixel = (tile.y0 + ((item >> 3) & 7u)) * Pt.W + tile.x0 + (item & 7u), rng.sample = Pt.sample_begin + pool_first + (item >> 6);
+			}
+			rng.block = 1u, rng.lobe_bits = Rng::spare22(w0, w2);
 			T = mk(1.0, 1.0, 1.0);
-			{
-				double u0, u1;
-				rng.next2(Pt.key0, Pt.key1, u0, u1);
-				primary_ray(Pt, x, y, u0, u1, ro, rd);
+			if (!emitter_item) {
+				primary_ray(Pt, tile.x0 + (item & 7u), tile.y0 + ((item >> 3) & 7u), Rng::to_unit(w0, w1), Rng::to_unit(w2, w3), ro, rd);
 				if (Pt.use_dof) failed = active && !thin_lens_from_pinhole(Pt, ro, rd, rng, ro, rd);
 			}
-			pairs = (uint32_t)__builtin_amdgcn_readfirstlane((int)item_sets[0]);
+			pairs = CLASSED ? head0 & ((1u << kTileClassShift) - 1u) : head0;
 			turns = (unsigned long long)(uint32_t)__builtin_amdgcn_readfirstlane((int)item_sets[1]) | (unsigned long long)(uint32_t)__builtin_amdgcn_readfirstlane((int)item_sets[2]) << 32;
+			if (CLASSED) turns = 0ull;
+			if (emitter_item) pairs = 0u;
 		}
 		const bool want = active && !failed;
 		double t = 0.0;
@@ -691,6 +821,37 @@
 				atomicAdd(&Pt.debug_counters[34], (unsigned long long)__popcll(dm)), atomicAdd(&Pt.debug_counters[35], (unsigned long long)__popcll(dropped));
 				atomicAdd(&Pt.debug_counters[36], pairs != Pt.axis_pairs ? 1ull : 0ull);
 			}
+		}
+#endif
+#if RMD_DIAG
+		if (__ballot(diag_emitter) != 0ull && (Pt.debug_flags & 512u) && (Pt.debug_flags & 8u) && Pt.debug_counters) {
+			const bool active = diag_emitter;
+			const int wall = __builtin_amdgcn_readfirstlane((int)item_sets[1]);
+			Rng r;
+			r.init(rng.pixel, rng.sample);
+			double u0, u1, t_full = 0.0;
+			uint32_t sub_full = 0;
+			V3 fro, frd;
+			r.next2(Pt.key0, Pt.key1, u0, u1);
+			primary_ray(Pt, tile.x0 + (item & 7u), tile.y0 + ((item >> 3) & 7u), u0, u1, fro, frd);
+			const int oi_full = scene_intersect_wave<false>(objs, Pt.n_objects, grids, nullptr, *no_scratch, active, fro, frd, t_full, sub_full, Pt.axis_pairs, 0u, nullptr, false, Pt.visit_mask);
+			bool bad_sample = true;
+			if (oi_full >= 0) {
+				const V3 c = hadamard(mk(1.0, 1.0, 1.0), ld3(lobjs[oi_full].color)), L = hadamard(T, ld3(lobjs[wall].color));
+				bad_sample = lobjs[oi_full].material_kind != 2u || __builtin_bit_cast(unsigned long long, c.x) != __builtin_bit_cast(unsigned long long, L.x) ||
+				             __builtin_bit_cast(unsigned long long, c.y) != __builtin_bit_cast(unsigned long long, L.y) || __builtin_bit_cast(unsigned long long, c.z) != __builtin_bit_cast(unsigned long long, L.z);
+			}
+			const unsigned long long cm = __ballot(active), bm = __ballot(active && bad_sample), om = __ballot(active && oi_full != wall);
+			if (lane == 0u) {
+				atomicAdd(&Pt.debug_counters[55], (unsigned long long)__popcll(cm)), atomicAdd(&Pt.debug_counters[56], (unsigned long long)__popcll(bm)), atomicAdd(&Pt.debug_counters[57], (unsigned long long)__popcll(om));
+				atomicAdd(&Pt.debug_counters[32], (unsigned long long)__popcll(cm)), atomicAdd(&Pt.debug_counters[34], (unsigned long long)__popcll(om));
+			}
+		}
+#endif
+#if RMD_DIAG
+		if (CLASSED && !shade_trip && (Pt.debug_flags & 512u) && (Pt.debug_flags & 8u) && Pt.debug_counters) {
+			const unsigned long long om = __ballot(want && oi != __builtin_amdgcn_readfirstlane((int)item_sets[1]));
+			if (lane == 0u) atomicAdd(&Pt.debug_counters[57], (unsigned long long)__popcll(om));
 		}
 #endif
 		bool terminal = failed, park = false, emitted = false;
@@ -750,6 +911,9 @@
 			__builtin_amdgcn_fence(__ATOMIC_ACQUIRE, "wavefront");
 		}
 	}
+	};
+	if ((uint32_t)__builtin_amdgcn_readfirstlane((int)item_sets[0]) >> kTileClassShift != kTileGeneral) trip_loop(std::true_type{});
+	else trip_loop(std::false_type{});
 	finish_sample_range<MOM>(P, tile, wt, P.split_k, work_item < P.n_whole, lane, out, out_sq);
 }
 
@@ -1176,6 +1340,11 @@
 		if ((tid & 63u) == 0u) *last_draw = 0u;
 		for (;;) {
 			uint32_t item = 0, floor = 0;
+			if constexpr (kSortedTrips<MODE, GRID>) {
+				unsigned char *area = wave_lds;
+				asm volatile("" : "+v"(area));
+				last_draw = reinterpret_cast<volatile uint32_t *>(area + wave_lds_of<MODE, GRID, QUEUED>(P.n_grids) - kWaveHeadBytes);
+			}
 			if ((tid & 63u) == 0u) {
 				item = atomicAdd(P.work_counter, 1u);
 				floor = *last_draw;
diff --git a/raymond_amd/probe.py b/raymond_amd/probe.py
--- a/raymond_amd/probe.py
+++ b/raymond_amd/probe.py
@@ -33,6 +33,7 @@
     "rmd_probe_triangle_sphere": [_sz, _vp, _vp],
     "rmd_probe_pretest_pairs": [_vp, _sz, _vp, _vp, _vp, _vp, _vp, _vp],
     "rmd_probe_primary_candidates": [_P(abi.Camera), _P(abi.Settings), _P(abi.Object), C.c_uint32, C.c_uint32, C.c_int64, _sz, _vp, _vp, _vp],
+    "rmd_probe_tile_classes": [_P(abi.Camera), _P(abi.Settings), _P(abi.Object), C.c_uint32, C.c_uint32, C.c_int64, _sz, _vp, _vp, _vp],
     "rmd_probe_launch_plan": [C.c_uint32, C.c_uint32, _sz, _vp, _vp],
     "rmd_probe_launch_sizes": [C.c_uint32, C.c_uint32, _vp],
     "rmd_probe_work_plan": [_vp, _sz, _vp, _vp],
@@ -213,6 +214,22 @@
     return int(launch[0]), int(launch[1]), bool(launch[2]), out[:, 0].copy(), out[:, 1].astype(np.uint32)
 
 
+TILE_GENERAL, TILE_EMITTER, TILE_BLACK = 0, 1, 2
+
+
+def tile_classes(cam, settings, scene, tiles, axis_pairs_tunable=0):
+    L = _L()
+    objs, n, _descs, ng, keep = scene.flatten()
+    tiles = np.ascontiguousarray(tiles, dtype=np.uint32).reshape(-1, 4)
+    launch, out = np.zeros(1, dtype=np.uint32), np.zeros((tiles.shape[0], 2), dtype=np.int32)
+    c, s = cam.pod(), settings.pod()
+    st = L.rmd_probe_tile_classes(C.byref(c), C.byref(s), objs, n, ng, int(axis_pairs_tunable), tiles.shape[0], _p(tiles), _p(launch), _p(out))
+    del keep
+    if st != abi.RMD_OK:
+        raise RuntimeError("rmd_probe_tile_classes: status %d" % st)
+    return bool(launch[0]), out[:, 0].copy(), out[:, 1].copy()
+
+
 MODE_TILES, MODE_TILES_BUFFERED, MODE_LIST = 0, 1, 2
 PLAN_QUEUES, PLAN_PERSIST, PLAN_CHAIN, PLAN_MOMENTS = 1, 2, 4, 8
 PLAN_FIELDS = ("persistent", "queued", "chained", "moments", "waves_per_wg", "workgroups", "wave_lds", "lds")
```

Measured after the change: 27360 (median of 6 runs). 1.03x the previous value.
